# cmaestre/pcl_tracking

Hardware: NVIDIA B200
Metric: likelihood evals/s (particle x model-point), 217k-pt scene tracker frame (higher is better)
Workload: dtype f32

## Files before the change

include/pft/pft.h:

```cpp
#ifndef PFT_PFT_H_
#define PFT_PFT_H_

#include <stddef.h>
#include <stdint.h>

#ifdef __cplusplus
extern "C" {
#endif

#define PFT_API __attribute__((visibility("default")))

typedef enum {
  PFT_OK = 0,
  PFT_ERR_INVALID = -1,
  PFT_ERR_CUDA = -2,
  PFT_ERR_STATE = -3,
  PFT_ERR_CAPACITY = -4,
  PFT_ERR_COMM = -5
} pft_status;

typedef struct { float x, y, z; uint32_t rgba; } pft_point;
typedef struct { float x, y, z, w; uint32_t rgba; uint32_t pad[3]; } pft_point_pcl32;
typedef struct { float x, y, z, one, roll, pitch, yaw, weight; } pft_particle;

// ... 50 lines not shown
  PFT_SAMPLER = 7,
  PFT_QUAT_SAMPLE = 8,
  PFT_USE_NORMAL = 9,
  PFT_MIN_INDICES = 10,
  PFT_DEBUG_NN = 11,
  PFT_CANDIDATE_LISTS = 12,
  PFT_USE_CHANGE_DETECTOR = 13,
  PFT_CHANGE_DETECTOR_INTERVAL = 14,
  PFT_CHANGE_DETECTOR_MIN_POINTS = 15,
  PFT_DELTA = 20,
  PFT_EPSILON = 21,
  PFT_ALPHA = 22,
  PFT_MOTION_RATIO = 23,
  PFT_MAX_DIST = 24,
  PFT_DIST_WEIGHT = 25,
  PFT_HSV_WEIGHT = 26,
  PFT_H_WEIGHT = 27, PFT_S_WEIGHT = 28, PFT_V_WEIGHT = 29,
  PFT_SEARCH_RESOLUTION = 30,
  PFT_RESAMPLE_LIKELIHOOD_THR = 31,
  PFT_CHANGE_DETECTOR_RESOLUTION = 32,
  PFT_STEP_NOISE_COV = 40,
  PFT_INIT_NOISE_COV = 41,
  PFT_INIT_NOISE_MEAN = 42,
  PFT_BIN_SIZE = 43
} pft_key;

typedef enum {
  PFT_NN_EXACT = 0,
  PFT_NN_PCL_APPROX = 1
} pft_nn_mode;
typedef enum { PFT_SAMPLER_ALIAS_PCL = 0, PFT_SAMPLER_CDF = 1, PFT_SAMPLER_CDF_VDC = 2 } pft_sampler;

PFT_API int pft_tracker_create(pft_context* ctx, int kld, pft_tracker** out);
PFT_API void pft_tracker_destroy(pft_tracker* t);
PFT_API int pft_tracker_set_i(pft_tracker* t, int key, int value);
PFT_API int pft_tracker_set_d(pft_tracker* t, int key, double value);
PFT_API int pft_tracker_set_vec6(pft_tracker* t, int key, const double* v6);
PFT_API int pft_tracker_set_trans(pft_tracker* t, const float* m12);
PFT_API int pft_tracker_set_reference_cloud(pft_tracker* t, const pft_cloud* cloud);
PFT_API int pft_tracker_set_reference_points(pft_tracker* t, const void* host_points, size_t n, int layout);
PFT_API int pft_tracker_set_input_cloud(pft_tracker* t, const pft_cloud* cloud);

PFT_API int pft_tracker_compute(pft_tracker* t);
PFT_API int pft_compute_batch(pft_tracker** trackers, int n);
PFT_API int pft_tracker_get_result(pft_tracker* t, pft_particle* out);
PFT_API int pft_tracker_get_particles(pft_tracker* t, pft_particle* out, size_t capacity, size_t* n);
PFT_API int pft_particle_to_matrix(pft_context* ctx, const pft_particle* p, float* m12);
typedef struct {
  float centroid[3];
  float axes[9];
  float extent[3];
  float center[3];
  float quat[4];
  float eigenvalues[3];
  int32_t n;
} pft_result_box;
PFT_API int pft_tracker_get_result_box(pft_tracker* t, float z_offset, pft_result_box* out);
PFT_API int pft_tracker_reset(pft_tracker* t);
PFT_API int pft_tracker_get_eval_count(pft_tracker* t, uint64_t* out);
PFT_API int pft_tracker_get_fit_ratio(pft_tracker* t, double* out);

PFT_API int pft_tracker_set_particles(pft_tracker* t, const pft_particle* p, size_t n);
PFT_API int pft_tracker_set_result(pft_tracker* t, const pft_particle* representative, const pft_particle* motion);
PFT_API int pft_tracker_get_motion(pft_tracker* t, pft_particle* out);
PFT_API int pft_tracker_inject_draws(pft_tracker* t, const float* u_select, const float* normals6,
                                     const float* u_motion, int slots, int stride);
PFT_API int pft_tracker_seed(pft_tracker* t, uint64_t seed);
PFT_API int pft_tracker_init_particles(pft_tracker* t);
PFT_API int pft_tracker_resample(pft_tracker* t, int slot);
PFT_API int pft_tracker_weight(pft_tracker* t);
PFT_API int pft_tracker_update(pft_tracker* t);
PFT_API int pft_tracker_set_changed(pft_tracker* t, int changed);
PFT_API int pft_tracker_get_change_detector_info(pft_tracker* t, int32_t* out4);
PFT_API int pft_tracker_get_aabb(pft_tracker* t, float* aabb6);
PFT_API int pft_tracker_get_cropped_count(pft_tracker* t, size_t* n);
PFT_API int pft_tracker_get_raw_weights(pft_tracker* t, float* out, size_t capacity, size_t* n);
PFT_API int pft_tracker_get_ancestors(pft_tracker* t, int32_t* out, size_t capacity, size_t* n);
PFT_API int pft_tracker_get_nn(pft_tracker* t, int particle, int32_t* idx, float* d2, size_t capacity);
PFT_API int pft_tracker_get_timing(pft_tracker* t, float* weight_kernel_ms, float* compute_ms);
PFT_API int pft_tracker_enable_timing(pft_tracker* t, int on);
PFT_API int pft_tracker_get_kernel_times(pft_tracker* t, const char** names, float* ms, int capacity, int* n);

PFT_API int pft_tracker_get_index_info(pft_tracker* t, int* info8);
PFT_API int pft_tracker_graph_replays(pft_tracker* t, uint64_t* n);

PFT_API int pft_tracker_weight_phase(pft_tracker* t, int phase);
PFT_API int pft_tracker_get_crop_box(pft_tracker* t, float* aabb6);
PFT_API int pft_tracker_set_crop_box(pft_tracker* t, const float* aabb6);
PFT_API int pft_tracker_get_raw_slice(pft_tracker* t, int rank, float* out, size_t capacity, size_t* n);
PFT_API int pft_tracker_set_raw_slice(pft_tracker* t, int rank, const float* in, size_t n);
PFT_API int pft_tracker_set_shard(pft_tracker* t, int nranks, int rank);

PFT_API int pft_comm_get_unique_id(void* id128);
PFT_API int pft_context_comm_init(pft_context* ctx, int nranks, int rank, const void* id128);
PFT_API int pft_context_comm_destroy(pft_context* ctx);
PFT_API int pft_cloud_broadcast(pft_cloud* cloud, size_t capacity, int root);
PFT_API int pft_tracker_comm_init(pft_tracker* t, int nranks, int rank, const void* id128);
PFT_API int pft_tracker_comm_destroy(pft_tracker* t);


#define PFT_PEER_HANDLE_BYTES 64
PFT_API int pft_tracker_peer_export(pft_tracker* t, void* handle64);
PFT_API int pft_tracker_peer_attach(pft_tracker* t, const void* handles );
PFT_API int pft_tracker_peer_detach(pft_tracker* t);

#define PFT_CLOUD_PEER_HANDLE_BYTES 192
PFT_API int pft_cloud_peer_export(pft_cloud* cloud, size_t capacity, void* handles192);
PFT_API int pft_cloud_peer_attach(pft_cloud* cloud, const void* handles , int nranks, int rank);
PFT_API int pft_cloud_peer_broadcast(pft_cloud* cloud, int root);
PFT_API int pft_cloud_peer_detach(pft_cloud* cloud);

PFT_API int pft_tracker_set_devices(pft_tracker* t, int n, const int* devices);
PFT_API int pft_tracker_get_follower(pft_tracker* t, int rank, pft_tracker** out);

#ifdef __cplusplus
}
#endif
#endif
```

pcl_tracking_b200/_capi.py:

```python
import ctypes as C
import os

import numpy as np

_HERE = os.path.dirname(os.path.abspath(__file__))
LIB_PATH = os.environ.get("PFT_LIB") or os.path.join(_HERE, "lib", "libpft.so")
HEADER_PATH = os.path.join(os.path.dirname(_HERE), "include", "pft", "pft.h")

POINT = np.dtype([("x", "<f4"), ("y", "<f4"), ("z", "<f4"), ("rgba", "<u4")])
POINT_PCL32 = np.dtype([("x", "<f4"), ("y", "<f4"), ("z", "<f4"), ("w", "<f4"), ("rgba", "<u4"), ("pad", "<u4", (3,))])
PARTICLE = np.dtype([("x", "<f4"), ("y", "<f4"), ("z", "<f4"), ("one", "<f4"),
                     ("roll", "<f4"), ("pitch", "<f4"), ("yaw", "<f4"), ("weight", "<f4")])

RESULT_BOX = np.dtype([("centroid", "<f4", (3,)), ("axes", "<f4", (3, 3)), ("extent", "<f4", (3,)), ("center", "<f4", (3,)),
                       ("quat", "<f4", (4,)), ("eigenvalues", "<f4", (3,)), ("n", "<i4")])

LAYOUT_PACKED16, LAYOUT_PCL32 = 0, 1
OK, ERR_INVALID, ERR_CUDA, ERR_STATE, ERR_CAPACITY, ERR_COMM = 0, -1, -2, -3, -4, -5

THREADS, PARTICLE_NUM, MAX_PARTICLE_NUM, ITERATION_NUM, NN_MODE, USE_HSV, USE_DISTANCE, SAMPLER, QUAT_SAMPLE, USE_NORMAL, MIN_INDICES, DEBUG_NN, CANDIDATE_LISTS = range(13)
(DELTA, EPSILON, ALPHA, MOTION_RATIO, MAX_DIST, DIST_WEIGHT, HSV_WEIGHT, H_WEIGHT, S_WEIGHT, V_WEIGHT, SEARCH_RESOLUTION,
 RESAMPLE_LIKELIHOOD_THR) = range(20, 32)
STEP_NOISE_COV, INIT_NOISE_COV, INIT_NOISE_MEAN, BIN_SIZE = range(40, 44)
USE_CHANGE_DETECTOR, CHANGE_DETECTOR_INTERVAL, CHANGE_DETECTOR_MIN_POINTS = 13, 14, 15
CHANGE_DETECTOR_RESOLUTION = 32
NN_EXACT, NN_PCL_APPROX = 0, 1
PEER_HANDLE_BYTES = 64
CLOUD_PEER_HANDLE_BYTES = 192
SAMPLER_ALIAS_PCL, SAMPLER_CDF, SAMPLER_CDF_VDC = 0, 1, 2


class PftError(RuntimeError):
    def __init__(self, code, msg):
        super().__init__("pft error %d: %s" % (code, msg))
        self.code = code


_vp, _i, _f, _d, _sz, _u64 = C.c_void_p, C.c_int, C.c_float, C.c_double, C.c_size_t, C.c_uint64
_pp = C.POINTER(C.c_void_p)
_psz = C.POINTER(C.c_size_t)

SIGNATURES = {
    "pft_last_error": (C.c_char_p, []),
    "pft_version": (C.c_char_p, []),
    "pft_device_count": (_i, []),
    "pft_context_create": (_i, [_i, _pp]),
    "pft_context_destroy": (None, [_vp]),
    "pft_context_synchronize": (_i, [_vp]),
    "pft_context_stream": (_vp, [_vp]),
    "pft_host_alloc": (_i, [_pp, _sz]),
    "pft_host_free": (_i, [_vp]),
    "pft_kernel_launch_count": (_u64, []),
    "pft_cloud_create": (_i, [_vp, _pp]),
    "pft_cloud_destroy": (None, [_vp]),
    "pft_cloud_upload": (_i, [_vp, _vp, _sz, _i]),
    "pft_cloud_upload_pointcloud2": (_i, [_vp, _vp, C.c_uint32, C.c_uint32, C.c_uint32, C.c_uint32, C.c_int32, C.c_int32, C.c_int32, C.c_int32, _i]),
    "pft_cloud_upload_async": (_i, [_vp, _vp, _sz, _i]),
    "pft_cloud_upload_pointcloud2_async": (_i, [_vp, _vp, C.c_uint32, C.c_uint32, C.c_uint32, C.c_uint32, C.c_int32, C.c_int32, C.c_int32, C.c_int32, _i]),
    "pft_cloud_wait_upload": (_i, [_vp]),
    "pft_cloud_size": (_i, [_vp, _psz]),
    "pft_cloud_download": (_i, [_vp, _vp, _sz, _i, _psz]),
    "pft_passthrough": (_i, [_vp, _vp, _vp, _i, _f, _f]),
    "pft_passthrough_voxel_grid": (_i, [_vp, _vp, _vp, _f, _i, _f, _f]),
    "pft_approx_voxel_grid_pcl": (_i, [_vp, _vp, _vp, _f, _i, _f, _f]),
    "pft_prepare_model": (_i, [_vp, _vp, _vp, _f, _vp]),
    "pft_euclidean_clusters": (_i, [_vp, _vp, _d, _i, _i, _vp, _sz, _vp, _sz, _psz]),
    "pft_cloud_select_cluster": (_i, [_vp, _vp, _i, _vp]),
    "pft_segment_plane": (_i, [_vp, _vp, _d, _i, _d, _vp, _i, _u64, _i, _vp, C.POINTER(C.c_int32), _vp, _vp, _psz]),
    "pft_tracker_create": (_i, [_vp, _i, _pp]),
    "pft_tracker_destroy": (None, [_vp]),
    "pft_tracker_set_i": (_i, [_vp, _i, _i]),
    "pft_tracker_set_d": (_i, [_vp, _i, _d]),
    "pft_tracker_set_vec6": (_i, [_vp, _i, _vp]),
    "pft_tracker_set_trans": (_i, [_vp, _vp]),
    "pft_tracker_set_reference_cloud": (_i, [_vp, _vp]),
    "pft_tracker_set_reference_points": (_i, [_vp, _vp, _sz, _i]),
    "pft_tracker_set_input_cloud": (_i, [_vp, _vp]),
    "pft_tracker_compute": (_i, [_vp]),
    "pft_compute_batch": (_i, [_pp, _i]),
    "pft_tracker_get_result": (_i, [_vp, _vp]),
    "pft_tracker_get_particles": (_i, [_vp, _vp, _sz, _psz]),
    "pft_particle_to_matrix": (_i, [_vp, _vp, _vp]),
    "pft_tracker_get_result_box": (_i, [_vp, _f, _vp]),
    "pft_tracker_reset": (_i, [_vp]),
    "pft_tracker_get_eval_count": (_i, [_vp, C.POINTER(C.c_uint64)]),
    "pft_tracker_get_fit_ratio": (_i, [_vp, C.POINTER(C.c_double)]),
    "pft_tracker_set_particles": (_i, [_vp, _vp, _sz]),
    "pft_tracker_set_result": (_i, [_vp, _vp, _vp]),
    "pft_tracker_get_motion": (_i, [_vp, _vp]),
    "pft_tracker_inject_draws": (_i, [_vp, _vp, _vp, _vp, _i, _i]),
    "pft_tracker_seed": (_i, [_vp, _u64]),
    "pft_tracker_init_particles": (_i, [_vp]),
    "pft_tracker_resample": (_i, [_vp, _i]),
    "pft_tracker_weight": (_i, [_vp]),
    "pft_tracker_update": (_i, [_vp]),
    "pft_tracker_set_changed": (_i, [_vp, _i]),
    "pft_tracker_get_change_detector_info": (_i, [_vp, _vp]),
    "pft_tracker_get_aabb": (_i, [_vp, _vp]),
    "pft_tracker_get_cropped_count": (_i, [_vp, _psz]),
    "pft_tracker_get_raw_weights": (_i, [_vp, _vp, _sz, _psz]),
    "pft_tracker_get_ancestors": (_i, [_vp, _vp, _sz, _psz]),
    "pft_tracker_get_nn": (_i, [_vp, _i, _vp, _vp, _sz]),
    "pft_tracker_get_timing": (_i, [_vp, C.POINTER(C.c_float), C.POINTER(C.c_float)]),
    "pft_tracker_enable_timing": (_i, [_vp, _i]),
    "pft_tracker_get_kernel_times": (_i, [_vp, _vp, _vp, _i, C.POINTER(C.c_int)]),
    "pft_tracker_get_index_info": (_i, [_vp, _vp]),
    "pft_tracker_graph_replays": (_i, [_vp, C.POINTER(C.c_uint64)]),
    "pft_tracker_weight_phase": (_i, [_vp, _i]),
    "pft_tracker_get_crop_box": (_i, [_vp, _vp]),
    "pft_tracker_set_crop_box": (_i, [_vp, _vp]),
    "pft_tracker_get_raw_slice": (_i, [_vp, _i, _vp, _sz, _psz]),
    "pft_tracker_set_raw_slice": (_i, [_vp, _i, _vp, _sz]),
    "pft_tracker_set_shard": (_i, [_vp, _i, _i]),
    "pft_comm_get_unique_id": (_i, [_vp]),
    "pft_context_comm_init": (_i, [_vp, _i, _i, _vp]),
    "pft_context_comm_destroy": (_i, [_vp]),
    "pft_cloud_broadcast": (_i, [_vp, _sz, _i]),
    "pft_tracker_comm_init": (_i, [_vp, _i, _i, _vp]),
    "pft_tracker_comm_destroy": (_i, [_vp]),
    "pft_cloud_peer_export": (_i, [_vp, _sz, _vp]),
    "pft_cloud_peer_attach": (_i, [_vp, _vp, _i, _i]),
    "pft_cloud_peer_broadcast": (_i, [_vp, _i]),
    "pft_cloud_peer_detach": (_i, [_vp]),
    "pft_tracker_set_devices": (_i, [_vp, _i, _vp]),
    "pft_tracker_get_follower": (_i, [_vp, _i, _vp]),
    "pft_tracker_peer_export": (_i, [_vp, _vp]),
    "pft_tracker_peer_attach": (_i, [_vp, _vp]),
    "pft_tracker_peer_detach": (_i, [_vp]),
}

_lib = None


def load():
    global _lib
    if _lib is None:
        if not os.path.exists(LIB_PATH):
            raise ImportError(
                "%s is missing: build it with `python -m pcl_tracking_b200.build` (nvcc, sm_100a). "
                "There is no CPU fallback." % LIB_PATH)
        L = C.CDLL(LIB_PATH)
        for name, (res, args) in SIGNATURES.items():
            fn = getattr(L, name)
            fn.restype = res
            fn.argtypes = args
        _lib = L
    return _lib


def check(rc):
    if rc != 0:
        raise PftError(rc, load().pft_last_error().decode("utf-8", "replace"))


def ptr(a):
    return a.ctypes.data_as(C.c_void_p)
```

pcl_tracking_b200/csrc/pft_filters.cu:

```cuda
#include <stdlib.h>
#include <string.h>

#include "pft_internal.h"

namespace pft {

namespace {

constexpr unsigned long long kEmptyKey = ~0ull;
constexpr int kFirstInit = 0x7f7f7f7f;

__device__ __forceinline__ bool finite3(const float4& p) { return isfinite(p.x) && isfinite(p.y) && isfinite(p.z); }

__device__ __forceinline__ bool passes(const float4& p, int field, float lo, float hi) {
  if (!finite3(p)) return false;
  if (field < 0) return true;
  const float v = field == 0 ? p.x : (field == 1 ? p.y : p.z);
  return !(v < lo || v > hi);
}

__device__ __forceinline__ unsigned long long voxel_key(const float4& p, float inv) {
  const int ix = (int)floorf(p.x * inv), iy = (int)floorf(p.y * inv), iz = (int)floorf(p.z * inv);
  const unsigned long long bx = (unsigned long long)((ix + (1 << 20)) & 0x1fffff);
  const unsigned long long by = (unsigned long long)((iy + (1 << 20)) & 0x1fffff);
  const unsigned long long bz = (unsigned long long)((iz + (1 << 20)) & 0x1fffff);
  return (bx << 42) | (by << 21) | bz;
}
__device__ __forceinline__ unsigned int hash_key(unsigned long long k) {
  k ^= k >> 33; k *= 0xff51afd7ed558ccdull; k ^= k >> 33; k *= 0xc4ceb9fe1a85ec53ull; k ^= k >> 33;
  return (unsigned int)k;
}

__global__ void unpack_pcl32_kernel(const uint4* __restrict__ src, float4* __restrict__ dst, size_t n) {
  for (size_t i = blockIdx.x * (size_t)blockDim.x + threadIdx.x; i < n; i += (size_t)gridDim.x * blockDim.x) {
    const uint4 a = src[2 * i];
    const uint4 b = src[2 * i + 1];
    dst[i] = make_float4(__uint_as_float(a.x), __uint_as_float(a.y), __uint_as_float(a.z), __uint_as_float(b.x));
  }
}
__global__ void pack_pcl32_kernel(const float4* __restrict__ src, uint4* __restrict__ dst, size_t n) {
  for (size_t i = blockIdx.x * (size_t)blockDim.x + threadIdx.x; i < n; i += (size_t)gridDim.x * blockDim.x) {
    const float4 p = src[i];
    dst[2 * i] = make_uint4(__float_as_uint(p.x), __float_as_uint(p.y), __float_as_uint(p.z), __float_as_uint(1.0f));
    dst[2 * i + 1] = make_uint4(__float_as_uint(p.w), 0u, 0u, 0u);
  }
}
__global__ void unpack_pointcloud2_kernel(const unsigned int* __restrict__ src, float4* __restrict__ dst, unsigned int width, unsigned int height,
                                          unsigned int point_words, unsigned int row_words, int wx, int wy, int wz, int wrgb) {
  const size_t n = (size_t)width * height;
  for (size_t i = blockIdx.x * (size_t)blockDim.x + threadIdx.x; i < n; i += (size_t)gridDim.x * blockDim.x) {
    const size_t row = i / width, col = i - row * width;
    const unsigned int* rec = src + row * row_words + col * point_words;
    const unsigned int rgba = wrgb >= 0 ? rec[wrgb] : 0u;
    dst[i] = make_float4(__uint_as_float(rec[wx]), __uint_as_float(rec[wy]), __uint_as_float(rec[wz]), __uint_as_float(rgba));
  }
}
__global__ void set_header_kernel(CloudHeader* h, int n) { h->n = n; }

__global__ void __launch_bounds__(1024) passthrough_kernel(const float4* __restrict__ in, const CloudHeader* __restrict__ in_hdr,
                                                           float4* __restrict__ out, CloudHeader* out_hdr, int field, float lo,
                                                           float hi, int drop_zero) {
  __shared__ int smem[34];
  const int n = in_hdr->n;
  auto keep = [&](int i) -> int {
    const float4 p = in[i];
    if (!passes(p, field, lo, hi)) return 0;
    if (drop_zero && fabs((double)p.x) < 0.01 && fabs((double)p.y) < 0.01 && fabs((double)p.z) < 0.01) return 0;
    return 1;
  };
  const int total = block_exclusive_scan<int>(
      n, keep, [&](int i, int ex) { const float4 p = in[i]; if (keep(i)) out[ex] = p; }, smem);
  if (threadIdx.x == 0) out_hdr->n = total;
}

__global__ void k1_insert_kernel(const float4* __restrict__ in, const CloudHeader* __restrict__ in_hdr, unsigned long long* keys,
                                 int* first, int* __restrict__ slot_of, unsigned int mask, float inv, int field, float lo, float hi) {
  const int n = in_hdr->n;
  for (int i = blockIdx.x * blockDim.x + threadIdx.x; i < n; i += gridDim.x * blockDim.x) {
    const float4 p = in[i];
    int slot = -1;
    if (passes(p, field, lo, hi)) {
      const unsigned long long key = voxel_key(p, inv);
      unsigned int s = hash_key(key) & mask;
      while (true) {
        const unsigned long long prev = atomicCAS(&keys[s], kEmptyKey, key);
        if (prev == kEmptyKey || prev == key) break;
        s = (s + 1) & mask;
      }
      slot = (int)s;
      atomicMin(&first[s], i);
    }
    slot_of[i] = slot;
  }
}
constexpr int kTile = 4096;

__device__ __forceinline__ int k1_is_first(int i, int n, const int* __restrict__ slot_of, const int* __restrict__ first) {
  if (i >= n) return 0;
  const int s = slot_of[i];
  return (s >= 0 && first[s] == i) ? 1 : 0;
}
__global__ void __launch_bounds__(1024) k1_tile_count_kernel(const CloudHeader* __restrict__ in_hdr, const int* __restrict__ slot_of,
                                                             const int* __restrict__ first, int* __restrict__ tile_count) {
  __shared__ int red[32];
  const int n = in_hdr->n;
  const int base = blockIdx.x * kTile + threadIdx.x * 4;
  int c = 0;
#pragma unroll
  for (int k = 0; k < 4; ++k) c += k1_is_first(base + k, n, slot_of, first);
  c = warp_sum(c);
  if ((threadIdx.x & 31) == 0) red[threadIdx.x >> 5] = c;
  __syncthreads();
  if (threadIdx.x < 32) {
    int v = red[threadIdx.x];
    v = warp_sum(v);
    if (threadIdx.x == 0) tile_count[blockIdx.x] = v;
  }
}
__global__ void __launch_bounds__(1024) k1_tile_scan_kernel(int n_tiles, int* tile_count, CloudHeader* out_hdr) {
  __shared__ int smem[34];
  const int total = block_exclusive_scan<int>(
      n_tiles, [&](int i) { return tile_count[i]; }, [&](int i, int ex) { tile_count[i] = ex; }, smem);
  if (threadIdx.x == 0) out_hdr->n = total;
}
__global__ void __launch_bounds__(1024) k1_tile_assign_kernel(const CloudHeader* __restrict__ in_hdr, const int* __restrict__ slot_of,
                                                              const int* __restrict__ first, const int* __restrict__ tile_offset,
                                                              int* __restrict__ vid, double* acc_xyz, unsigned int* acc_rgbc) {
  __shared__ int wsum[32];
  const int n = in_hdr->n;
  const int lane = threadIdx.x & 31, wid = threadIdx.x >> 5;
  const int base = blockIdx.x * kTile + threadIdx.x * 4;
  int f[4], sum = 0;
#pragma unroll
  for (int k = 0; k < 4; ++k) { f[k] = k1_is_first(base + k, n, slot_of, first); sum += f[k]; }
  int inc = sum;
#pragma unroll
  for (int o = 1; o < 32; o <<= 1) { const int t = __shfl_up_sync(kFull, inc, o); if (lane >= o) inc += t; }
  if (lane == 31) wsum[wid] = inc;
  __syncthreads();
  if (wid == 0) {
    const int w = wsum[lane];
    int winc = w;
#pragma unroll
    for (int o = 1; o < 32; o <<= 1) { const int t = __shfl_up_sync(kFull, winc, o); if (lane >= o) winc += t; }
    wsum[lane] = winc - w;
  }
  __syncthreads();
  int ex = tile_offset[blockIdx.x] + wsum[wid] + (inc - sum);
#pragma unroll
  for (int k = 0; k < 4; ++k) {
    if (f[k]) {
      vid[slot_of[base + k]] = ex;
      ++ex;
    }
  }
}
__global__ void k1_accum_kernel(const float4* __restrict__ in, const CloudHeader* __restrict__ in_hdr, const int* __restrict__ slot_of,
                                const int* __restrict__ vid, double* acc_xyz, unsigned int* acc_rgbc) {
  const int n = in_hdr->n;
  for (int i = blockIdx.x * blockDim.x + threadIdx.x; i < n; i += gridDim.x * blockDim.x) {
    const int s = slot_of[i];
    if (s < 0) continue;
    const int v = vid[s];
    const float4 p = in[i];
    const unsigned int rgba = __float_as_uint(p.w);
    atomicAdd(&acc_xyz[3 * v], (double)p.x);
    atomicAdd(&acc_xyz[3 * v + 1], (double)p.y);
    atomicAdd(&acc_xyz[3 * v + 2], (double)p.z);
    atomicAdd(&acc_rgbc[4 * v], (rgba >> 16) & 0xffu);
    atomicAdd(&acc_rgbc[4 * v + 1], (rgba >> 8) & 0xffu);
    atomicAdd(&acc_rgbc[4 * v + 2], rgba & 0xffu);
    atomicAdd(&acc_rgbc[4 * v + 3], 1u);
  }
}
__global__ void k1_final_kernel(const CloudHeader* __restrict__ out_hdr, const double* __restrict__ acc_xyz,
                                const unsigned int* __restrict__ acc_rgbc, float4* __restrict__ out) {
  const int n = out_hdr->n;
  for (int v = blockIdx.x * blockDim.x + threadIdx.x; v < n; v += gridDim.x * blockDim.x) {
    const uint4 c = reinterpret_cast<const uint4*>(acc_rgbc)[v];
    const double cnt = (double)c.w;
    const float fc = (float)c.w;
    const unsigned int r = (unsigned int)(int)((float)c.x / fc), g = (unsigned int)(int)((float)c.y / fc), b = (unsigned int)(int)((float)c.z / fc);
    out[v] = make_float4((float)(acc_xyz[3 * v] / cnt), (float)(acc_xyz[3 * v + 1] / cnt), (float)(acc_xyz[3 * v + 2] / cnt),
                         __uint_as_float((r << 16) | (g << 8) | b));
  }
}

__global__ void approx_voxel_grid_pcl_kernel(const float4* __restrict__ in, const CloudHeader* __restrict__ in_hdr, float inv, int field, float lo,
                                             float hi, float4* __restrict__ out, CloudHeader* out_hdr) {
  if (threadIdx.x != 0 || blockIdx.x != 0) return;
  constexpr int kHist = 512;
  __shared__ int s_key[kHist][4];
  __shared__ float s_acc[kHist][6];
  for (int k = 0; k < kHist; ++k) { s_key[k][3] = 0; for (int q = 0; q < 6; ++q) s_acc[k][q] = 0.f; }
  const int n = in_hdr->n;
  int op = 0;
  auto flush = [&](int k) {
    const float cnt = (float)s_key[k][3];
    const unsigned int r = (unsigned int)(int)(s_acc[k][3] / cnt), g = (unsigned int)(int)(s_acc[k][4] / cnt), b = (unsigned int)(int)(s_acc[k][5] / cnt);
    out[op++] = make_float4(s_acc[k][0] / cnt, s_acc[k][1] / cnt, s_acc[k][2] / cnt, __uint_as_float((r << 16) | (g << 8) | b));
  };
  for (int i = 0; i < n; ++i) {
    const float4 p = in[i];
    if (!passes(p, field, lo, hi)) continue;
    const int ix = (int)floorf(p.x * inv), iy = (int)floorf(p.y * inv), iz = (int)floorf(p.z * inv);
    const int k = (int)((unsigned int)(ix * 7171 + iy * 3079 + iz * 4231) & (unsigned int)(kHist - 1));
    if (s_key[k][3] && (ix != s_key[k][0] || iy != s_key[k][1] || iz != s_key[k][2])) {
      flush(k);
      s_key[k][3] = 0;
      for (int q = 0; q < 6; ++q) s_acc[k][q] = 0.f;
    }
    s_key[k][0] = ix; s_key[k][1] = iy; s_key[k][2] = iz; s_key[k][3]++;
    const unsigned int rgba = __float_as_uint(p.w);
    s_acc[k][0] += p.x; s_acc[k][1] += p.y; s_acc[k][2] += p.z;
    s_acc[k][3] += (float)((rgba >> 16) & 0xffu); s_acc[k][4] += (float)((rgba >> 8) & 0xffu); s_acc[k][5] += (float)(rgba & 0xffu);
  }
  for (int k = 0; k < kHist; ++k) if (s_key[k][3]) flush(k);
  out_hdr->n = op;
}

__global__ void __launch_bounds__(1024) centre_kernel(float4* pts, const CloudHeader* __restrict__ hdr, float* centroid3) {
  __shared__ double red[32];
  __shared__ float c[3];
  const int n = hdr->n;
  double sx = 0, sy = 0, sz = 0;
  for (int i = threadIdx.x; i < n; i += blockDim.x) { const float4 p = pts[i]; sx += (double)p.x; sy += (double)p.y; sz += (double)p.z; }
  sx = block_sum(sx, red); sy = block_sum(sy, red); sz = block_sum(sz, red);
  if (threadIdx.x == 0) {
    const double dn = n > 0 ? (double)n : 1.0;
    c[0] = (float)(sx / dn); c[1] = (float)(sy / dn); c[2] = (float)(sz / dn);
    centroid3[0] = c[0]; centroid3[1] = c[1]; centroid3[2] = c[2];
  }
  __syncthreads();
  for (int i = threadIdx.x; i < n; i += blockDim.x) { float4 p = pts[i]; p.x = p.x - c[0]; p.y = p.y - c[1]; p.z = p.z - c[2]; pts[i] = p; }
}

inline int grid_for(size_t n, int block, int sm_count) {
  size_t g = (n + block - 1) / block;
  size_t cap = (size_t)sm_count * 8;
  if (g > cap) g = cap;
  if (g < 1) g = 1;
  return (int)g;
}

}

int launch_unpack_pcl32(cudaStream_t s, const void* src32, float4* dst, size_t n) {
  if (n == 0) return PFT_OK;
  unpack_pcl32_kernel<<<grid_for(n, 256, 148), 256, 0, s>>>(reinterpret_cast<const uint4*>(src32), dst, n);
  PFT_LAUNCH_CHECK();
  return PFT_OK;
}
int launch_unpack_pointcloud2(cudaStream_t s, const void* src, float4* dst, unsigned int width, unsigned int height, unsigned int point_step,
                              unsigned int row_step, int off_x, int off_y, int off_z, int off_rgb) {
  const size_t n = (size_t)width * height;
  if (n == 0) return PFT_OK;
  unpack_pointcloud2_kernel<<<grid_for(n, 256, 148), 256, 0, s>>>(reinterpret_cast<const unsigned int*>(src), dst, width, height, point_step / 4, row_step / 4,
                                                                 off_x / 4, off_y / 4, off_z / 4, off_rgb >= 0 ? off_rgb / 4 : -1);
  PFT_LAUNCH_CHECK();
  return PFT_OK;
}
int launch_pack_pcl32(cudaStream_t s, const float4* src, void* dst32, size_t n) {
  if (n == 0) return PFT_OK;
  pack_pcl32_kernel<<<grid_for(n, 256, 148), 256, 0, s>>>(src, reinterpret_cast<uint4*>(dst32), n);
  PFT_LAUNCH_CHECK();
  return PFT_OK;
}
int launch_set_header(cudaStream_t s, CloudHeader* hdr, int n) {
  set_header_kernel<<<1, 1, 0, s>>>(hdr, n);
  PFT_LAUNCH_CHECK();
  return PFT_OK;
}

int run_passthrough(pft_context* ctx, const pft_cloud* in, pft_cloud* out, int field, float lo, float hi, int drop_zero) {
  int rc = out->ensure(in->capacity);
  if (rc) return rc;
  passthrough_kernel<<<1, 1024, 0, ctx->stream>>>(in->d_pts(), in->d_hdr(), out->d_pts(), out->d_hdr(), field, lo, hi, drop_zero);
  PFT_LAUNCH_CHECK();
  out->host_n = -1;
  return PFT_OK;
}

static int enqueue_voxel_grid(pft_context* ctx, const pft_cloud* in, pft_cloud* out, float leaf, int field, float lo, float hi, size_t cap, size_t H,
                              int n_tiles) {
  cudaStream_t s = ctx->stream;
  PFT_CUDA_TRY(cudaMemsetAsync(ctx->k1_keys.p, 0xff, H * sizeof(unsigned long long), s));
  PFT_CUDA_TRY(cudaMemsetAsync(ctx->k1_first.p, 0x7f, H * sizeof(int), s));
  PFT_CUDA_TRY(cudaMemsetAsync(ctx->k1_acc_xyz.p, 0, cap * 3 * sizeof(double), s));
  PFT_CUDA_TRY(cudaMemsetAsync(ctx->k1_acc_rgbc.p, 0, cap * 4 * sizeof(unsigned int), s));
  const float inv = 1.0f / leaf;
  const int grid = grid_for(cap, 256, ctx->sm_count);
  k1_insert_kernel<<<grid, 256, 0, s>>>(in->d_pts(), in->d_hdr(), ctx->k1_keys.as<unsigned long long>(), ctx->k1_first.as<int>(),
                                        ctx->k1_slot_of.as<int>(), (unsigned int)(H - 1), inv, field, lo, hi);
  PFT_LAUNCH_CHECK();
  k1_tile_count_kernel<<<n_tiles, 1024, 0, s>>>(in->d_hdr(), ctx->k1_slot_of.as<int>(), ctx->k1_first.as<int>(), ctx->k1_blk.as<int>());
  PFT_LAUNCH_CHECK();
  k1_tile_scan_kernel<<<1, 1024, 0, s>>>(n_tiles, ctx->k1_blk.as<int>(), out->d_hdr());
  PFT_LAUNCH_CHECK();
  k1_tile_assign_kernel<<<n_tiles, 1024, 0, s>>>(in->d_hdr(), ctx->k1_slot_of.as<int>(), ctx->k1_first.as<int>(), ctx->k1_blk.as<int>(),
                                                 ctx->k1_vid.as<int>(), ctx->k1_acc_xyz.as<double>(), ctx->k1_acc_rgbc.as<unsigned int>());
  PFT_LAUNCH_CHECK();
  k1_accum_kernel<<<grid, 256, 0, s>>>(in->d_pts(), in->d_hdr(), ctx->k1_slot_of.as<int>(), ctx->k1_vid.as<int>(),
                                       ctx->k1_acc_xyz.as<double>(), ctx->k1_acc_rgbc.as<unsigned int>());
  PFT_LAUNCH_CHECK();
  k1_final_kernel<<<grid, 256, 0, s>>>(out->d_hdr(), ctx->k1_acc_xyz.as<double>(), ctx->k1_acc_rgbc.as<unsigned int>(), out->d_pts());
  PFT_LAUNCH_CHECK();
  return PFT_OK;
}

int run_voxel_grid(pft_context* ctx, const pft_cloud* in, pft_cloud* out, float leaf, int field, float lo, float hi) {
  if (!(leaf > 0.f)) { set_last_error("leaf size must be positive"); return PFT_ERR_INVALID; }
  const size_t cap = in->capacity;
  int rc = out->ensure(cap);
  if (rc) return rc;
  if (cap == 0) return launch_set_header(ctx->stream, out->d_hdr(), 0);
  size_t H = 1024;
  while (H < 2 * cap) H <<= 1;
  if ((rc = ctx->k1_keys.reserve(H * sizeof(unsigned long long)))) return rc;
  if ((rc = ctx->k1_first.reserve(H * sizeof(int)))) return rc;
  if ((rc = ctx->k1_vid.reserve(H * sizeof(int)))) return rc;
  if ((rc = ctx->k1_slot_of.reserve(cap * sizeof(int)))) return rc;
  if ((rc = ctx->k1_acc_xyz.reserve(cap * 3 * sizeof(double)))) return rc;
  if ((rc = ctx->k1_acc_rgbc.reserve(cap * 4 * sizeof(unsigned int)))) return rc;
  const int n_tiles = (int)((cap + kTile - 1) / kTile);
  if ((rc = ctx->k1_blk.reserve((size_t)n_tiles * sizeof(int)))) return rc;
  out->host_n = -1;
  (void)kFirstInit;
  static const bool use_graph = [] { const char* e = getenv("PFT_NO_GRAPH"); return !(e && e[0] == '1'); }();
  if (!use_graph) return enqueue_voxel_grid(ctx, in, out, leaf, field, lo, hi, cap, H, n_tiles);
  pft_context::K1Key key;
  memset(&key, 0, sizeof(key));
  key.p[0] = in->d_pts(); key.p[1] = in->d_hdr(); key.p[2] = out->d_pts(); key.p[3] = out->d_hdr();
  key.p[4] = ctx->k1_keys.p; key.p[5] = ctx->k1_first.p; key.p[6] = ctx->k1_vid.p; key.p[7] = ctx->k1_slot_of.p;
  key.p[8] = ctx->k1_acc_xyz.p; key.p[9] = ctx->k1_acc_rgbc.p; key.p[10] = ctx->k1_blk.p;
  key.cap = cap; key.H = H; key.leaf = leaf; key.lo = lo; key.hi = hi; key.field = field;
  int slot = -1;
  for (int k = 0; k < pft_context::kK1Graphs; ++k)
    if (ctx->k1_exec[k] && memcmp(&ctx->k1_key[k], &key, sizeof(key)) == 0) { slot = k; break; }
  if (slot < 0) {
    slot = ctx->k1_next;
    ctx->k1_next = (ctx->k1_next + 1) % pft_context::kK1Graphs;
    if (ctx->k1_exec[slot]) { cudaGraphExecDestroy(ctx->k1_exec[slot]); ctx->k1_exec[slot] = nullptr; }
    cudaGraph_t graph = nullptr;
    const unsigned long long before = g_launch_count.load();
    PFT_CUDA_TRY(cudaStreamBeginCapture(ctx->stream, cudaStreamCaptureModeThreadLocal));
    rc = enqueue_voxel_grid(ctx, in, out, leaf, field, lo, hi, cap, H, n_tiles);
    cudaError_t ce = cudaStreamEndCapture(ctx->stream, &graph);
    g_launch_count -= g_launch_count.load() - before;
    if (rc) { if (graph) cudaGraphDestroy(graph); return rc; }
    if (ce != cudaSuccess) { set_last_error("downsample graph capture failed: %s", cudaGetErrorString(ce)); cudaGetLastError(); return PFT_ERR_CUDA; }
    cudaError_t ie = cudaGraphInstantiate(&ctx->k1_exec[slot], graph, 0);
    cudaGraphDestroy(graph);
    if (ie != cudaSuccess) { set_last_error("downsample graph instantiate failed: %s", cudaGetErrorString(ie)); cudaGetLastError(); ctx->k1_exec[slot] = nullptr; return PFT_ERR_CUDA; }
    ctx->k1_key[slot] = key;
  }
  PFT_CUDA_TRY(cudaGraphLaunch(ctx->k1_exec[slot], ctx->stream));
  g_launch_count += 6;
  return PFT_OK;
}

int run_approx_voxel_grid_pcl(pft_context* ctx, const pft_cloud* in, pft_cloud* out, float leaf, int field, float lo, float hi) {
  if (!(leaf > 0.f)) { set_last_error("leaf size must be positive"); return PFT_ERR_INVALID; }
  int rc = out->ensure(in->capacity);
  if (rc) return rc;
  approx_voxel_grid_pcl_kernel<<<1, 32, 0, ctx->stream>>>(in->d_pts(), in->d_hdr(), 1.0f / leaf, field, lo, hi, out->d_pts(), out->d_hdr());
  PFT_LAUNCH_CHECK();
  out->host_n = -1;
  return PFT_OK;
}

int run_centre_on_centroid(pft_context* ctx, pft_cloud* cloud, float* d_centroid3) {
  centre_kernel<<<1, 1024, 0, ctx->stream>>>(cloud->d_pts(), cloud->d_hdr(), d_centroid3);
  PFT_LAUNCH_CHECK();
  return PFT_OK;
}

}
```

pcl_tracking_b200/csrc/pft_tracker.cu:

```cuda
#include <dlfcn.h>
#include <math.h>
#include <stdio.h>
#include <stdlib.h>
#include <string.h>

#include <algorithm>
#include <vector>

#include "pft_internal.h"
#include "pft_tracker_kernels.cuh"

using namespace pft;

namespace {

struct UidByValue { char internal[128]; };
struct NcclApi {
  void* lib = nullptr;
  bool tried = false;
  int (*GetUniqueId)(void*) = nullptr;
  int (*CommInitRank)(void**, int, UidByValue, int) = nullptr;
  int (*CommDestroy)(void*) = nullptr;
  int (*AllGather)(const void*, void*, size_t, int, void*, cudaStream_t) = nullptr;
  int (*Broadcast)(const void*, void*, size_t, int, int, void*, cudaStream_t) = nullptr;
// ... 23 lines not shown
  g_nccl.GetUniqueId = (decltype(g_nccl.GetUniqueId))sym("ncclGetUniqueId");
  g_nccl.CommInitRank = (decltype(g_nccl.CommInitRank))sym("ncclCommInitRank");
  g_nccl.CommDestroy = (decltype(g_nccl.CommDestroy))sym("ncclCommDestroy");
  g_nccl.AllGather = (decltype(g_nccl.AllGather))sym("ncclAllGather");
  g_nccl.AllReduce = (decltype(g_nccl.AllReduce))sym("ncclAllReduce");
  g_nccl.Broadcast = (decltype(g_nccl.Broadcast))sym("ncclBroadcast");
  g_nccl.GroupStart = (decltype(g_nccl.GroupStart))sym("ncclGroupStart");
  g_nccl.GroupEnd = (decltype(g_nccl.GroupEnd))sym("ncclGroupEnd");
  g_nccl.GetErrorString = (decltype(g_nccl.GetErrorString))sym("ncclGetErrorString");
  if (!g_nccl.GetUniqueId || !g_nccl.CommInitRank || !g_nccl.CommDestroy || !g_nccl.AllGather || !g_nccl.AllReduce || !g_nccl.Broadcast || !g_nccl.GroupStart ||
      !g_nccl.GroupEnd) {
    set_last_error("NCCL library lacks a required symbol");
    return PFT_ERR_COMM;
  }
  g_nccl.lib = h;
  return PFT_OK;
}
#define PFT_NCCL_TRY(expr)                                                                                       \
  do {                                                                                                           \
    int _r = (expr);                                                                                             \
    if (_r != 0) {                                                                                               \
      set_last_error("%s:%d: %s -> %s", __FILE__, __LINE__, #expr, g_nccl.GetErrorString ? g_nccl.GetErrorString(_r) : "nccl error"); \
      return PFT_ERR_COMM;                                                                                       \
    }                                                                                                            \
  } while (0)

inline int blocks_for(long long n, int block, int cap) {
  long long g = (n + block - 1) / block;
  if (g > cap) g = cap;
  if (g < 1) g = 1;
  return (int)g;
}

}

struct pft_tracker {
  pft_context* ctx = nullptr;
  bool kld = true;
  int threads = 0, particle_num = 0, max_particle_num = 0, iteration_num = 1, min_indices = 1;
  int nn_mode = PFT_NN_EXACT, use_hsv = 0, use_dist = 1, sampler = PFT_SAMPLER_CDF, quat_sample = 1, debug_nn = 0;
  double delta = 0.99, epsilon = 0.0, alpha = 15.0, motion_ratio = 0.25, max_dist = 1.79769313486231570815e+308;
  double dist_w = 1.0, hsv_w = 1.0, h_w = 1.0, s_w = 1.0, v_w = 0.0, search_res = 0.01, resample_thr = 0.0;
  double step_cov[6] = {0, 0, 0, 0, 0, 0}, init_cov[6] = {0, 0, 0, 0, 0, 0}, init_mean[6] = {0, 0, 0, 0, 0, 0};
  float bin_size[6] = {0, 0, 0, 0, 0, 0};
  float trans[12] = {1, 0, 0, 0, 0, 1, 0, 0, 0, 0, 1, 0};
  unsigned long long seed = 0x5eedull;
  bool changed = false, has_particles = false;
  int n_cap = 0;
  int M = 0;
  const pft_cloud* input = nullptr;
  size_t scene_cap = 0;
  int max_cells = 1 << 20;
  int list_mode = 1;
  int list_max_cells = 1 << 19;
  int cur = 0;
  int inj_slots = 0, inj_stride = 0;
  int draw_cap = 0;
  bool timing = false;
  float t_weight_ms = 0.f, t_compute_ms = 0.f;
  std::vector<cudaEvent_t> ev_w;
  cudaEvent_t ev_c0 = nullptr, ev_c1 = nullptr;
  int n_ev_used = 0;
  std::vector<cudaEvent_t> ev_k;
  std::vector<const char*> ev_k_name;
  int n_ev_k = 0;
  void* comm = nullptr;
  int nranks = 1, rank = 0;
  bool peer_mode = false;
  bool peer_ipc = true;
  struct Follower { pft_context* ctx = nullptr; pft_tracker* t = nullptr; pft_cloud* scene = nullptr; pft_cloud* model = nullptr; cudaEvent_t scene_ready = nullptr, scene_free = nullptr; bool free_recorded = false; };
  std::vector<Follower> followers;
  bool md_attached = false, md_prepared = false;
  void* peer_local = nullptr;
  size_t peer_bytes = 0;
  PeerSet peers{};
  bool graph_enabled = true;
  cudaGraphExec_t graph_exec[2] = {nullptr, nullptr};
  const void* graph_scene_pts[2] = {nullptr, nullptr};
  const void* graph_scene_hdr[2] = {nullptr, nullptr};
  unsigned long long config_version = 1, graph_version[2] = {0, 0};
  unsigned long long graph_replays = 0;
  int graph_nodes[2] = {0, 0};
  DevBuf st, parts[2], mats, slot_aabb, model, model_perm, model_tmp, sort_keys, sort_idx, bbox, raw, partial, cdf, cdf_total, ancestors, bin_keys, tbl_rep,
      tbl_min, slot_of, klb, d_usel, d_normals, d_umot, idx_hdr, idx_hdr_prev, fbuilt_bits, cell_start, ipts, ipts2, ihsv, icount, dbg_idx, dbg_d2, d_trans, row_table, flists, fpool, fcell_items, fl1_slots, fneeded, fneeded_list, ffar_list, xlists, xcount, result_box, alias_a, alias_q, alias_hl, oct_hdr, oct_nodes, oct_next, cd_hdr, cd_nodes, cd_out;
  int oct_node_cap = 0;
  bool use_cd = false;
  int cd_interval = 10, cd_filter = 10, change_counter = 0, cd_tests = 0, cd_last_found = -1, cd_node_cap = 0, cd_resets = 0;
  double cd_res = 0.01;
  int lists_smem = 0;
  int tbl_size = 0;
  int n_slots = 0;
  int chunks = 1, chunk_len = 0;

  cudaStream_t aux_stream = nullptr;
  cudaEvent_t ev_fork = nullptr, ev_join = nullptr;
  cudaStream_t batch_stream = nullptr;
  cudaEvent_t batch_done = nullptr;
  bool batch_active = false;

  int slice_cap() const { return (n_cap + nranks - 1) / nranks; }
  cudaStream_t run_stream() const { return batch_active ? batch_stream : ctx->stream; }
};

namespace {

void invalidate_graph(pft_tracker* t) { t->config_version++; }

void stage_mark(pft_tracker* t, const char* name) {
  if (!t->timing) return;
  if ((int)t->ev_k.size() <= t->n_ev_k) {
    cudaEvent_t e;
    if (cudaEventCreate(&e) != cudaSuccess) return;
    t->ev_k.push_back(e);
    t->ev_k_name.push_back(name);
  }
  t->ev_k_name[t->n_ev_k] = name;
  cudaEventRecord(t->ev_k[t->n_ev_k++], t->run_stream());
}

void release_all(pft_tracker* t) {
  DevBuf* bufs[] = {&t->st, &t->parts[0], &t->parts[1], &t->mats, &t->slot_aabb, &t->model, &t->model_perm, &t->model_tmp, &t->sort_keys, &t->sort_idx,
                    &t->bbox, &t->raw, &t->partial, &t->cdf, &t->cdf_total, &t->ancestors, &t->bin_keys, &t->tbl_rep, &t->tbl_min, &t->slot_of, &t->klb,
                    &t->d_usel, &t->d_normals, &t->d_umot, &t->idx_hdr, &t->idx_hdr_prev, &t->fbuilt_bits, &t->cell_start, &t->ipts, &t->ipts2, &t->ihsv, &t->icount, &t->dbg_idx,
                    &t->dbg_d2, &t->d_trans, &t->row_table, &t->flists, &t->fpool, &t->fcell_items, &t->fl1_slots, &t->fneeded, &t->fneeded_list, &t->ffar_list, &t->xlists, &t->xcount, &t->result_box, &t->alias_a, &t->alias_q, &t->alias_hl, &t->oct_hdr, &t->oct_nodes, &t->oct_next, &t->cd_hdr, &t->cd_nodes, &t->cd_out};
  for (auto* b : bufs) b->release();
}

NoiseParams make_noise(const pft_tracker* t, const double* mean, const double* cov) {
  NoiseParams np;
  for (int d = 0; d < 6; ++d) { np.mean[d] = mean[d]; np.sigma[d] = sqrt(cov[d]); }
  const float scale_factor = 0.2862f;
  for (int d = 0; d < 3; ++d) np.sigma_q[d] = sqrt((double)scale_factor * cov[3 + d]);
  np.quat_mode = t->quat_sample;
  return np;
}

double normal_quantile(double u) {
  static const double a[9] = {1.24818987e-4, -1.075204047e-3, 5.198775019e-3, -0.019198292004, 0.059054035642,
                              -0.151968751364, 0.319152932694, -0.5319230073, 0.797884560593};
  static const double b[15] = {-4.5255659e-5, 1.5252929e-4, -1.9538132e-5, -6.76904986e-4, 1.390604284e-3,
                               -7.9462082e-4, -2.034254874e-3, 6.549791214e-3, -0.010557625006, 0.011630447319,
                               -9.279453341e-3, 5.353579108e-3, -2.141268741e-3, 5.35310549e-4, 0.999936657524};
  if (u == 0.) return 0.5;
  double y = u / 2.0, z;
  if (y < -3.) return 0.0;
  if (y > 3.) return 1.0;
  if (y < 0.0) y = -y;
  if (y < 1.0) {
    const double w = y * y;
    z = a[0];
    for (int i = 1; i < 9; i++) z = z * w + a[i];
    z *= (y * 2.0);
  } else {
    y -= 2.0;
    z = b[0];
    for (int i = 1; i < 15; i++) z = z * y + b[i];
  }
  return u < 0.0 ? (1.0 - z) / 2.0 : (1.0 + z) / 2.0;
}
double kl_bound(int k, double delta, double eps) {
  const double z = normal_quantile(delta);
  const double chi = 1.0 - 2.0 / (9.0 * (k - 1)) + sqrt(2.0 / (9.0 * (k - 1))) * z;
  return ((k - 1.0) / (2.0 * eps)) * chi * chi * chi;
}

constexpr long long kMarkCountMaxQueries = 16ll << 20;
constexpr int kClusterMinParticles = 4096;
constexpr int kListThreads = 640;
constexpr int kListThreadsBig = 896;
constexpr long long kListBigQueries = 48ll << 20;
constexpr long long kDynItemsPerWarp = 5;
constexpr int kItemsPerWarp = 6;
constexpr int kChunkWarpsPerSm = 24;
constexpr float kIndexDilate = 0.03f;
constexpr int kListRatio = 2;

template <typename... P, typename... A>
void launch_replicated(const pft_tracker* t, void (*one)(P...), void (*cluster)(P...), A... args) {
  if (t->n_cap > kClusterMinParticles) cluster<<<kClusterCtas, 1024, 0, t->run_stream()>>>(args...);
  else one<<<1, 1024, 0, t->run_stream()>>>(args...);
}

int upload_row_table(pft_tracker* t) {
  std::vector<RowEntry> tab;
  tab.reserve(kRows);
  for (int dz = -kRT; dz <= kRT; ++dz)
    for (int dy = -kRT; dy <= kRT; ++dy) {
      const int gy = std::max(std::abs(dy) - 1, 0), gz = std::max(std::abs(dz) - 1, 0);
      tab.push_back(RowEntry{(signed char)dy, (signed char)dz, (unsigned short)(gy * gy + gz * gz)});
    }
  std::stable_sort(tab.begin(), tab.end(), [](const RowEntry& a, const RowEntry& b) {
    if (a.lb2 != b.lb2) return a.lb2 < b.lb2;
    return (a.dy * a.dy + a.dz * a.dz) < (b.dy * b.dy + b.dz * b.dz);
  });
  int rc = t->row_table.reserve(tab.size() * sizeof(RowEntry));
  if (rc) return rc;
  PFT_CUDA_TRY(cudaMemcpyAsync(t->row_table.p, tab.data(), tab.size() * sizeof(RowEntry), cudaMemcpyHostToDevice, t->run_stream()));
  PFT_CUDA_TRY(cudaStreamSynchronize(t->run_stream()));
  int dev = t->ctx->device, max_optin = 0;
  PFT_CUDA_TRY(cudaDeviceGetAttribute(&max_optin, cudaDevAttrMaxSharedMemoryPerBlockOptin, dev));
  cudaFuncAttributes fa;
  PFT_CUDA_TRY(cudaFuncGetAttributes(&fa, weight_lists_kernel<true, kListThreads, true>));
  int dyn_l = (max_optin - (int)fa.sharedSizeBytes - 1024) & ~15;
  if (dyn_l < 0) dyn_l = 0;
  PFT_CUDA_TRY(cudaFuncSetAttribute(weight_lists_kernel<true, kListThreads, true>, cudaFuncAttributeMaxDynamicSharedMemorySize, dyn_l));
  PFT_CUDA_TRY(cudaFuncSetAttribute(weight_lists_kernel<true, kListThreads, false>, cudaFuncAttributeMaxDynamicSharedMemorySize, dyn_l));
  PFT_CUDA_TRY(cudaFuncSetAttribute(weight_lists_kernel<false, kListThreads, true>, cudaFuncAttributeMaxDynamicSharedMemorySize, dyn_l));
  PFT_CUDA_TRY(cudaFuncSetAttribute(weight_lists_kernel<false, kListThreads, false>, cudaFuncAttributeMaxDynamicSharedMemorySize, dyn_l));
  PFT_CUDA_TRY(cudaFuncSetAttribute(weight_lists_kernel<true, kListThreadsBig, true>, cudaFuncAttributeMaxDynamicSharedMemorySize, dyn_l));
  PFT_CUDA_TRY(cudaFuncSetAttribute(weight_lists_kernel<false, kListThreadsBig, true>, cudaFuncAttributeMaxDynamicSharedMemorySize, dyn_l));
  t->lists_smem = dyn_l;
  if (t->list_max_cells / 8 + 64 > max_optin - 2048) t->list_max_cells = (max_optin - 4096) * 8;
  PFT_CUDA_TRY(cudaFuncSetAttribute(cand_mark_kernel<false>, cudaFuncAttributeMaxDynamicSharedMemorySize, t->list_max_cells / 8 + 64));
  PFT_CUDA_TRY(cudaFuncSetAttribute(cand_mark_kernel<true>, cudaFuncAttributeMaxDynamicSharedMemorySize, t->list_max_cells / 8 + 64));
  return PFT_OK;
}

int upload_kl_table(pft_tracker* t);

int wanted_cap(const pft_tracker* t) { return t->kld ? std::max(t->max_particle_num, t->particle_num) : t->particle_num; }

int ensure_particle_buffers(pft_tracker* t) {
  const int cap = std::max(wanted_cap(t), t->n_cap);
  if (cap <= 0) { set_last_error("particle count is zero: call setParticleNum / setMaximumParticleNum first"); return PFT_ERR_STATE; }
  cudaStream_t s = t->run_stream();
  int rc;
  if (!t->st.p) {
    if ((rc = t->st.reserve(sizeof(TrackerState)))) return rc;
    PFT_CUDA_TRY(cudaMemsetAsync(t->st.p, 0, sizeof(TrackerState), s));
    DevParticle one{0.f, 0.f, 0.f, 1.f, 0.f, 0.f, 0.f, 0.f};
    PFT_CUDA_TRY(cudaMemcpyAsync(&t->st.as<TrackerState>()->rep, &one, sizeof(one), cudaMemcpyHostToDevice, s));
    PFT_CUDA_TRY(cudaMemcpyAsync(&t->st.as<TrackerState>()->motion, &one, sizeof(one), cudaMemcpyHostToDevice, s));
    PFT_CUDA_TRY(cudaStreamSynchronize(s));
    if ((rc = t->cdf_total.reserve(sizeof(unsigned long long)))) return rc;
    if ((rc = t->idx_hdr.reserve(sizeof(IndexHeader)))) return rc;
    if ((rc = t->idx_hdr_prev.reserve(sizeof(IndexHeader)))) return rc;
    PFT_CUDA_TRY(cudaMemsetAsync(t->idx_hdr.p, 0, sizeof(IndexHeader), s));
    PFT_CUDA_TRY(cudaMemsetAsync(t->idx_hdr_prev.p, 0, sizeof(IndexHeader), s));
    PFT_CUDA_TRY(cudaStreamSynchronize(s));
    if ((rc = t->d_trans.reserve(12 * sizeof(float)))) return rc;
    if ((rc = t->cell_start.reserve(((size_t)t->max_cells + 16) * sizeof(int)))) return rc;
    if ((rc = t->icount.reserve(((size_t)t->max_cells + 16) * sizeof(int)))) return rc;
    if ((rc = upload_row_table(t))) return rc;
    if (t->list_max_cells > 0) {
      if ((rc = t->flists.reserve(((size_t)t->list_max_cells + 1) * 8 * 8 * sizeof(unsigned int)))) return rc;
      if ((rc = t->fpool.reserve((size_t)kPoolGroups * 8 * sizeof(unsigned int)))) return rc;
      if ((rc = t->fcell_items.reserve(((size_t)t->list_max_cells + 16) * sizeof(int2)))) return rc;
      if ((rc = t->fl1_slots.reserve(((size_t)t->list_max_cells + 1) * kL1Cap * sizeof(unsigned short)))) return rc;
      if ((rc = t->fneeded.reserve(((size_t)t->list_max_cells + 16) * sizeof(unsigned int)))) return rc;
      if ((rc = t->fbuilt_bits.reserve(((size_t)t->list_max_cells / 32 + 16) * sizeof(unsigned int)))) return rc;
      if ((rc = t->fneeded_list.reserve(((size_t)t->list_max_cells / 2 + 4096) * sizeof(int)))) return rc;
      if ((rc = t->ffar_list.reserve(((size_t)t->list_max_cells + 16) * sizeof(int)))) return rc;
      if ((rc = t->xlists.reserve((size_t)kListXCells * kListKX * sizeof(unsigned int)))) return rc;
      if ((rc = t->xcount.reserve(64))) return rc;
    }
  }
  if (cap == t->n_cap) return PFT_OK;
  if (t->peer_local) {
    set_last_error("the particle capacity (%d -> %d) cannot change once the peer window is exported", t->n_cap, cap);
    return PFT_ERR_STATE;
  }
  invalidate_graph(t);
  PFT_CUDA_TRY(cudaStreamSynchronize(s));
  const int old_cap = t->n_cap;
  DevBuf np0, np1;
  if ((rc = np0.reserve((size_t)cap * sizeof(DevParticle)))) return rc;
  if ((rc = np1.reserve((size_t)cap * sizeof(DevParticle)))) return rc;
  if (old_cap > 0 && t->has_particles) {
    PFT_CUDA_TRY(cudaMemcpyAsync(np0.p, t->parts[t->cur].p, (size_t)std::min(cap, old_cap) * sizeof(DevParticle), cudaMemcpyDeviceToDevice, s));
    PFT_CUDA_TRY(cudaStreamSynchronize(s));
  }
  t->parts[0].release(); t->parts[1].release();
  t->parts[0] = np0; t->parts[1] = np1; t->cur = 0;
  t->n_cap = cap;
  t->n_slots = cap;
  const int slice = t->slice_cap();
  if ((rc = t->mats.reserve((size_t)cap * 12 * sizeof(float)))) return rc;
  t->slot_aabb.release();
  if ((rc = t->slot_aabb.reserve((size_t)cap * 6 * sizeof(float)))) return rc;
  {
    std::vector<float> init((size_t)cap * 6);
    for (int i = 0; i < cap; ++i) { for (int d = 0; d < 3; ++d) { init[6 * i + d] = FLT_MAX; init[6 * i + 3 + d] = -FLT_MAX; } }
    PFT_CUDA_TRY(cudaMemcpyAsync(t->slot_aabb.p, init.data(), init.size() * sizeof(float), cudaMemcpyHostToDevice, s));
    PFT_CUDA_TRY(cudaStreamSynchronize(s));
  }
  if ((rc = t->raw.reserve((size_t)slice * t->nranks * sizeof(float)))) return rc;
  PFT_CUDA_TRY(cudaMemsetAsync(t->raw.p, 0, (size_t)slice * t->nranks * sizeof(float), s));
  if ((rc = t->cdf.reserve((size_t)cap * sizeof(unsigned long long)))) return rc;
  if ((rc = t->ancestors.reserve((size_t)cap * sizeof(int)))) return rc;
  PFT_CUDA_TRY(cudaMemsetAsync(t->ancestors.p, 0xff, (size_t)cap * sizeof(int), s));
  PFT_CUDA_TRY(cudaStreamSynchronize(s));
  if (t->kld) {
    if ((rc = t->bin_keys.reserve((size_t)cap * 6 * sizeof(int)))) return rc;
    int ts = 1024;
    while (ts < 2 * cap) ts <<= 1;
    t->tbl_size = ts;
    if ((rc = t->tbl_rep.reserve((size_t)ts * sizeof(int)))) return rc;
    if ((rc = t->tbl_min.reserve((size_t)ts * sizeof(int)))) return rc;
    if ((rc = t->slot_of.reserve((size_t)cap * sizeof(int)))) return rc;
    if ((rc = t->klb.reserve((size_t)(cap + 2) * sizeof(double)))) return rc;
    if ((rc = upload_kl_table(t))) return rc;
  }
  return PFT_OK;
}

int upload_kl_table(pft_tracker* t) {
  if (!t->kld) return PFT_OK;
  const int n = t->n_cap + 2;
  std::vector<double> tab(n, 0.0);
  for (int k = 2; k < n; ++k) tab[k] = kl_bound(k, t->delta, t->epsilon);
  PFT_CUDA_TRY(cudaMemcpyAsync(t->klb.p, tab.data(), tab.size() * sizeof(double), cudaMemcpyHostToDevice, t->run_stream()));
  PFT_CUDA_TRY(cudaStreamSynchronize(t->run_stream()));
  return PFT_OK;
}

int ensure_draw_buffers(pft_tracker* t, int slots, int stride) {
  const size_t n = (size_t)slots * stride;
  int rc;
  if ((rc = t->d_usel.reserve(n * sizeof(float)))) return rc;
  if ((rc = t->d_normals.reserve(n * 6 * sizeof(float)))) return rc;
  if ((rc = t->d_umot.reserve(n * sizeof(float)))) return rc;
  return PFT_OK;
}

int reserve_generated_draws(pft_tracker* t, int count) {
  if (t->draw_cap >= count) return PFT_OK;
  int rc = ensure_draw_buffers(t, 1, count);
  if (rc) return rc;
  t->draw_cap = count;
  invalidate_graph(t);
  return PFT_OK;
}

int prepare_draws(pft_tracker* t, int slot, int count, const float** usel, const float** normals, const float** umot) {
  cudaStream_t s = t->run_stream();
  if (t->inj_stride > 0) {
    if (slot >= t->inj_slots || count > t->inj_stride) {
      set_last_error("injected draws cover %d slots x %d, need slot %d x %d", t->inj_slots, t->inj_stride, slot, count);
      return PFT_ERR_STATE;
    }
    *usel = t->d_usel.as<float>() + (size_t)slot * t->inj_stride;
    *normals = t->d_normals.as<float>() + (size_t)slot * t->inj_stride * 6;
    *umot = t->d_umot.as<float>() + (size_t)slot * t->inj_stride;
    return PFT_OK;
  }
  int rc = reserve_generated_draws(t, count);
  if (rc) return rc;
  draws_kernel<<<blocks_for(count, 256, t->ctx->sm_count * 4), 256, 0, s>>>(t->st.as<TrackerState>(), t->d_usel.as<float>(), t->d_normals.as<float>(),
                                                                        t->d_umot.as<float>(), count, t->seed);
  PFT_LAUNCH_CHECK();
  stage_mark(t, "draws_kernel");
  *usel = t->d_usel.as<float>(); *normals = t->d_normals.as<float>(); *umot = t->d_umot.as<float>();
  return PFT_OK;
}

int ensure_index_buffers(pft_tracker* t) {
  const size_t cap = std::max<size_t>(t->input ? t->input->capacity : 0, 1);
  if (cap <= t->scene_cap) return PFT_OK;
  invalidate_graph(t);
  PFT_CUDA_TRY(cudaStreamSynchronize(t->run_stream()));
  int rc;
  if ((rc = t->ipts.reserve((cap + 4) * sizeof(float4)))) return rc;
  if ((rc = t->ipts2.reserve((cap + 4) * sizeof(float4)))) return rc;
  if ((rc = t->ihsv.reserve((cap + 4) * sizeof(unsigned int)))) return rc;
  t->scene_cap = cap;
  return PFT_OK;
}

void choose_chunks(pft_tracker* t) {
  const int n_expected = std::max(1, (t->particle_num > 0 ? t->particle_num : t->n_cap) / t->nranks);
  const int total_warps = t->ctx->sm_count * kChunkWarpsPerSm;
  const int target_items = total_warps * kItemsPerWarp;
  const int max_chunks = std::max(1, (t->M + 63) / 64);
  int chunks = (target_items + n_expected - 1) / n_expected;
  chunks = std::min(std::max(chunks, 1), std::min(max_chunks, 256));
  int len = (t->M + chunks - 1) / chunks;
  len = ((len + 31) / 32) * 32;
  if (len < 32) len = 32;
  chunks = std::max(1, (t->M + len - 1) / len);
  if (chunks != t->chunks || len != t->chunk_len) invalidate_graph(t);
  t->chunks = chunks;
  t->chunk_len = len;
}

CoherenceParams make_coherence(const pft_tracker* t) {
  CoherenceParams c;
  c.max_d2 = t->max_dist * t->max_dist;
  c.dist_w = t->dist_w; c.hsv_w = t->hsv_w;
  c.h_w = (float)t->h_w; c.s_w = (float)t->s_w; c.v_w = (float)t->v_w;
  c.r_max = (float)std::min(t->max_dist, 1.0e18);
  c.use_dist = t->use_dist; c.use_hsv = t->use_hsv;
  return c;
}

int stage_init_particles(pft_tracker* t) {
  int rc = ensure_particle_buffers(t);
  if (rc) return rc;
  if (t->particle_num <= 0) { set_last_error("setParticleNum was not called"); return PFT_ERR_STATE; }
  if ((rc = upload_kl_table(t))) return rc;
  cudaStream_t s = t->run_stream();
  PFT_CUDA_TRY(cudaMemcpyAsync(t->d_trans.p, t->trans, sizeof(t->trans), cudaMemcpyHostToDevice, s));
  const float *usel, *normals, *umot;
  if ((rc = prepare_draws(t, 0, t->particle_num, &usel, &normals, &umot))) return rc;
  const NoiseParams np = make_noise(t, t->init_mean, t->init_cov);
  init_particles_kernel<<<blocks_for(t->particle_num, 128, 1 << 20), 128, 0, s>>>(t->st.as<TrackerState>(), t->parts[t->cur].as<DevParticle>(),
                                                                                   t->particle_num, t->d_trans.as<float>(), np, normals);
  PFT_LAUNCH_CHECK();
  stage_mark(t, "init_particles_kernel");
  t->has_particles = true;
  return PFT_OK;
}

int stage_resample(pft_tracker* t, int slot) {
  if (!t->has_particles) { set_last_error("resample before particles exist"); return PFT_ERR_STATE; }
  if (!t->input) { set_last_error("resample needs an input cloud (setInputCloud)"); return PFT_ERR_STATE; }
  if (t->kld && t->max_particle_num <= 0) { set_last_error("KLD tracker: setMaximumParticleNum was not called"); return PFT_ERR_STATE; }
  cudaStream_t s = t->run_stream();
  const int count = t->kld ? t->max_particle_num : t->particle_num;
  const float *usel = nullptr, *normals = nullptr, *umot = nullptr;
  int rc = PFT_OK;
  if (t->inj_stride > 0 && (rc = prepare_draws(t, slot, count, &usel, &normals, &umot))) return rc;
  TrackerState* st = t->st.as<TrackerState>();
  const DevParticle* old_parts = t->parts[t->cur].as<DevParticle>();
  DevParticle* new_parts = t->parts[t->cur ^ 1].as<DevParticle>();
  launch_replicated(t, cdf_kernel<1>, cdf_kernel<kClusterCtas>, st, old_parts, t->cdf.as<unsigned long long>(), t->cdf_total.as<unsigned long long>(),
                    t->tbl_rep.as<int>(), t->tbl_min.as<int>(), t->kld ? t->tbl_size : 0, t->kld ? 0 : t->particle_num, t->input->d_hdr());
  PFT_LAUNCH_CHECK();
  stage_mark(t, "cdf_kernel");
  if (t->sampler == PFT_SAMPLER_ALIAS_PCL) {
    alias_table_kernel<<<1, 32, 0, s>>>(st, old_parts, t->alias_a.as<int>(), t->alias_q.as<double>(), t->alias_hl.as<int>());
    PFT_LAUNCH_CHECK();
    stage_mark(t, "alias_table_kernel");
  }
  ResampleArgs a;
  a.alias_a = t->alias_a.as<int>(); a.alias_q = t->alias_q.as<double>();
  a.st = st; a.old_parts = old_parts; a.new_parts = new_parts;
  a.cdf = t->cdf.as<unsigned long long>(); a.cdf_total = t->cdf_total.as<unsigned long long>();
  a.u_select = usel; a.normals = normals; a.u_motion = umot; a.seed = t->seed;
  a.scene_hdr = t->input->d_hdr();
  a.ancestors = t->ancestors.as<int>(); a.bin_keys = t->bin_keys.as<int>();
  const double zero[6] = {0, 0, 0, 0, 0, 0};
  a.np = make_noise(t, zero, t->step_cov);
  a.motion_ratio = t->motion_ratio;
  for (int d = 0; d < 6; ++d) a.bin_size[d] = t->bin_size[d];
  a.kld = t->kld ? 1 : 0; a.n_max = t->max_particle_num; a.sampler = t->sampler; a.n_target = t->particle_num;
  resample_kernel<<<blocks_for(count, 128, t->ctx->sm_count * 16), 128, 0, s>>>(a);
  PFT_LAUNCH_CHECK();
// ... 14 lines not shown
int check_weight_ready(pft_tracker* t) {
  if (!t->has_particles) { set_last_error("weight before particles exist"); return PFT_ERR_STATE; }
  if (!t->input) { set_last_error("weight needs an input cloud (setInputCloud)"); return PFT_ERR_STATE; }
  if (t->M <= 0) { set_last_error("weight needs a reference cloud (setReferenceCloud)"); return PFT_ERR_STATE; }
  return ensure_index_buffers(t);
}

int weight_phase_box(pft_tracker* t) {
  int rc = check_weight_ready(t);
  if (rc) return rc;
  cudaStream_t s = t->run_stream();
  const int sm = t->ctx->sm_count;
  TrackerState* st = t->st.as<TrackerState>();
  DevParticle* parts = t->parts[t->cur].as<DevParticle>();
  matrices_kernel<<<blocks_for(t->n_cap, 128, sm * 8), 128, 0, s>>>(st, parts, t->mats.as<float>());
  PFT_LAUNCH_CHECK();
  stage_mark(t, "matrices_kernel");
  if (t->n_slots <= sm * 32) {
    aabb_kernel<4><<<std::min(t->n_slots, sm * 16), 128, 0, s>>>(st, t->model.as<float4>(), t->M, t->mats.as<float>(), t->slot_aabb.as<float>(), t->n_slots,
                                                                t->nranks, t->rank, t->peers, t->peer_mode ? 1 : 0);
  } else {
    aabb_kernel<1><<<std::min(t->n_slots, sm * 64), 32, 0, s>>>(st, t->model.as<float4>(), t->M, t->mats.as<float>(), t->slot_aabb.as<float>(), t->n_slots,
                                                               t->nranks, t->rank, t->peers, t->peer_mode ? 1 : 0);
  }
  PFT_LAUNCH_CHECK();
  stage_mark(t, "aabb_kernel");
  return PFT_OK;
}

bool nccl_exchange(const pft_tracker* t) { return t->comm && !t->peer_mode; }
bool normalize_sums_partials(const pft_tracker* t) { return t->nranks == 1 || t->peer_mode; }

int weight_comm_box(pft_tracker* t) {
  cudaStream_t s = t->run_stream();
  TrackerState* st = t->st.as<TrackerState>();
  PFT_NCCL_TRY(g_nccl.GroupStart());
  PFT_NCCL_TRY(g_nccl.AllReduce(st->aabb, st->aabb, 3, kNcclFloat, kNcclMin, t->comm, s));
  PFT_NCCL_TRY(g_nccl.AllReduce(st->aabb + 3, st->aabb + 3, 3, kNcclFloat, kNcclMax, t->comm, s));
  PFT_NCCL_TRY(g_nccl.GroupEnd());
  return PFT_OK;
}

template <typename Launch>
int timed_lookup(pft_tracker* t, const char* name, Launch launch) {
  cudaStream_t s = t->run_stream();
  if (t->timing) {
    while ((int)t->ev_w.size() < 2 * (t->n_ev_used + 1)) { cudaEvent_t e; PFT_CUDA_TRY(cudaEventCreate(&e)); t->ev_w.push_back(e); }
    PFT_CUDA_TRY(cudaEventRecord(t->ev_w[2 * t->n_ev_used], s));
  }
  launch();
  PFT_LAUNCH_CHECK();
  stage_mark(t, name);
  if (t->timing) { PFT_CUDA_TRY(cudaEventRecord(t->ev_w[2 * t->n_ev_used + 1], s)); t->n_ev_used++; }
  return PFT_OK;
}

int launch_raw_weights(pft_tracker* t) {
  const int local_cap = t->slice_cap();
  raw_weights_kernel<<<blocks_for(local_cap, 256, t->ctx->sm_count * 4), 256, 0, t->run_stream()>>>(
      t->st.as<TrackerState>(), t->partial.as<double>(), t->chunks, t->n_cap, t->raw.as<float>(), local_cap, t->nranks, t->rank);
  PFT_LAUNCH_CHECK();
  stage_mark(t, "raw_weights_kernel");
  return PFT_OK;
}

int weight_eval_pcl_approx(pft_tracker* t) {
  cudaStream_t s = t->run_stream();
  const int sm = t->ctx->sm_count;
  TrackerState* st = t->st.as<TrackerState>();
  const pft_cloud* in = t->input;
  octree_build_kernel<<<1, 32, 0, s>>>(in->d_pts(), in->d_hdr(), t->idx_hdr.as<IndexHeader>(), t->search_res, t->oct_nodes.as<OctNodeD>(), t->oct_node_cap,
                                       t->oct_next.as<int>(), t->oct_hdr.as<OctHeaderD>());
  PFT_LAUNCH_CHECK();
  stage_mark(t, "octree_build_kernel");
  WeightApproxArgs w;
  w.st = st; w.oct = t->oct_hdr.as<OctHeaderD>(); w.nodes = t->oct_nodes.as<OctNodeD>(); w.next = t->oct_next.as<int>();
  w.scene = in->d_pts(); w.model = t->model.as<float4>(); w.model_perm = t->model_perm.as<int>(); w.M = t->M; w.mats = t->mats.as<float>();
  w.partial = t->partial.as<double>(); w.chunks = t->chunks; w.chunk_len = t->chunk_len; w.n_max = t->n_cap; w.nranks = t->nranks; w.rank_id = t->rank;
  w.co = make_coherence(t);
  w.dbg_k = t->debug_nn; w.dbg_idx = t->dbg_idx.as<int>(); w.dbg_d2 = t->dbg_d2.as<float>();
  return timed_lookup(t, "weight_approx_kernel", [&] { weight_approx_kernel<<<sm * 8, 256, 0, s>>>(w); });
}

int launch_index_begin(pft_tracker* t, bool reuse_allowed = false) {
  const int sm = t->ctx->sm_count;
  const float inv_leaf = 1.0f / (float)t->search_res;
  index_begin_kernel<<<sm, 256, 0, t->run_stream()>>>(t->st.as<TrackerState>(), t->idx_hdr.as<IndexHeader>(), t->icount.as<int>(), inv_leaf, t->max_cells,
                                                      t->list_mode ? t->list_max_cells : 0, t->list_mode == 2 ? 0 : t->M, t->nranks, t->rank,
                                                      t->fneeded.as<unsigned int>(), t->xcount.as<int>(), t->fbuilt_bits.as<unsigned int>(),
                                                      reuse_allowed ? 1 : 0, t->iteration_num > 1 ? kIndexDilate : 0.f, kListRatio, t->idx_hdr_prev.as<IndexHeader>());
  PFT_LAUNCH_CHECK();
  stage_mark(t, "index_begin_kernel");
  return PFT_OK;
}

int weight_phase_eval(pft_tracker* t, bool reuse_allowed = false) {
  int rc = check_weight_ready(t);
  if (rc) return rc;
  cudaStream_t s = t->run_stream();
  const int sm = t->ctx->sm_count;
  TrackerState* st = t->st.as<TrackerState>();
  const pft_cloud* in = t->input;
  const int ncap_scene = (int)std::max<size_t>(in->capacity, 1);
  IndexHeader* hdr = t->idx_hdr.as<IndexHeader>();
  const float inv_leaf = 1.0f / (float)t->search_res;
  const int gscene = blocks_for(ncap_scene, 256, sm * 4);
  const bool lists = t->list_max_cells > 0 && t->list_mode && t->nn_mode == PFT_NN_EXACT;
  if ((rc = launch_index_begin(t, reuse_allowed && lists))) return rc;
  if (lists) {
    cudaStream_t sa = t->aux_stream;
    PFT_CUDA_TRY(cudaEventRecord(t->ev_fork, s));
    PFT_CUDA_TRY(cudaStreamWaitEvent(sa, t->ev_fork, 0));
    const long long n_queries = (long long)std::max(1, (t->particle_num > 0 ? t->particle_num : t->n_cap) / t->nranks) * t->M;
    const size_t mark_smem = (size_t)(t->list_max_cells / 8 + 64);
    if (n_queries <= kMarkCountMaxQueries) cand_mark_kernel<true><<<sm * 3, 256, mark_smem, sa>>>(st, hdr, t->model.as<float4>(), t->M, t->mats.as<float>(), t->fneeded.as<unsigned int>(), t->nranks, t->rank, t->fbuilt_bits.as<unsigned int>());
    else cand_mark_kernel<false><<<sm * 3, 256, mark_smem, sa>>>(st, hdr, t->model.as<float4>(), t->M, t->mats.as<float>(), t->fneeded.as<unsigned int>(), t->nranks, t->rank, t->fbuilt_bits.as<unsigned int>());
    PFT_LAUNCH_CHECK();
    cand_collect_kernel<<<sm * 2, 256, 0, sa>>>(hdr, t->fneeded.as<unsigned int>(), t->fneeded_list.as<int>(), t->xcount.as<int>());
    PFT_LAUNCH_CHECK();
    PFT_CUDA_TRY(cudaEventRecord(t->ev_join, sa));
  }
  index_count_kernel<<<gscene, 256, 0, s>>>(in->d_pts(), in->d_hdr(), hdr, t->icount.as<int>(), t->ipts2.as<float4>());
  PFT_LAUNCH_CHECK();
  stage_mark(t, "index_count_kernel");
  index_scan_kernel<<<1, 1024, 0, s>>>(hdr, t->icount.as<int>(), t->cell_start.as<int>(), st, t->ipts.as<float4>(), t->ipts2.as<float4>(), t->idx_hdr_prev.as<IndexHeader>());
  PFT_LAUNCH_CHECK();
  stage_mark(t, "index_scan_kernel");
  index_scatter_kernel<<<gscene, 256, 0, s>>>(in->d_pts(), in->d_hdr(), hdr, t->cell_start.as<int>(), t->icount.as<int>(), t->ipts.as<float4>(),
                                              t->ihsv.as<unsigned int>(), t->ipts2.as<float4>());
  PFT_LAUNCH_CHECK();
  stage_mark(t, "index_scatter_kernel");
  if (lists) {
    PFT_CUDA_TRY(cudaStreamWaitEvent(s, t->ev_join, 0));
    stage_mark(t, "cand_mark+collect (beside the index)");
    cand_build_kernel<<<sm * 8, 256, 0, s>>>(hdr, t->cell_start.as<int>(), t->ipts.as<float4>(), t->max_dist * t->max_dist, t->flists.as<unsigned int>(),
                                            t->fneeded.as<unsigned int>(), t->fneeded_list.as<int>(), t->xcount.as<int>(), t->ffar_list.as<int>(),
                                            t->fcell_items.as<int2>(), t->fl1_slots.as<unsigned short>(), t->fbuilt_bits.as<unsigned int>());
    PFT_LAUNCH_CHECK();
    stage_mark(t, "cand_build_kernel");
    cand_build_far_kernel<<<sm * 4, 256, 0, s>>>(hdr, t->cell_start.as<int>(), t->ipts.as<float4>(), t->max_dist * t->max_dist,
                                                t->flists.as<unsigned int>(), t->xlists.as<unsigned int>(), t->xcount.as<int>(), t->ffar_list.as<int>(),
                                                t->fneeded.as<unsigned int>(), t->fcell_items.as<int2>(), t->fl1_slots.as<unsigned short>(), t->fbuilt_bits.as<unsigned int>());
    PFT_LAUNCH_CHECK();
    stage_mark(t, "cand_build_far_kernel");
    cand_octant_kernel<<<sm * 8, 256, 0, s>>>(hdr, t->ipts.as<float4>(), t->max_dist * t->max_dist, t->flists.as<unsigned int>(), t->fpool.as<unsigned int>(),
                                             t->xcount.as<int>(), t->fcell_items.as<int2>(), t->fl1_slots.as<unsigned short>());
    PFT_LAUNCH_CHECK();
    stage_mark(t, "cand_octant_kernel");
  }
  if (t->nn_mode == PFT_NN_PCL_APPROX) return weight_eval_pcl_approx(t);
  WeightArgs a;
  a.st = st; a.hdr = hdr; a.pts2 = t->ipts2.as<float4>();
  a.flists = t->flists.as<unsigned int>(); a.pool = t->fpool.as<unsigned int>(); a.xlists = t->xlists.as<unsigned int>();
  a.cell_start = t->cell_start.as<int>(); a.pts = t->ipts.as<float4>();
  a.hsv = t->ihsv.as<unsigned int>(); a.table = t->row_table.as<RowEntry>(); a.smem_bytes = t->lists_smem;
  a.model = t->model.as<float4>(); a.model_perm = t->model_perm.as<int>(); a.M = t->M;
  a.mats = t->mats.as<float>();
  a.partial = t->partial.as<double>(); a.chunks = t->chunks; a.chunk_len = t->chunk_len; a.n_max = t->n_cap;
  a.nranks = t->nranks; a.rank_id = t->rank;
  a.co = make_coherence(t);
  a.dbg_k = t->debug_nn; a.dbg_idx = t->dbg_idx.as<int>(); a.dbg_d2 = t->dbg_d2.as<float>();
  const int wgrid = sm;
  const long long n_local = std::max(1, (t->particle_num > 0 ? t->particle_num : t->n_cap) / t->nranks);
  const bool dyn = n_local * t->chunks >= kDynItemsPerWarp * sm * (kListThreads / 32);
  return timed_lookup(t, "weight_lists_kernel", [&] {
    if (n_local * t->M >= kListBigQueries) {
      if (t->use_hsv) weight_lists_kernel<true, kListThreadsBig, true><<<wgrid, kListThreadsBig, t->lists_smem, s>>>(a);
      else weight_lists_kernel<false, kListThreadsBig, true><<<wgrid, kListThreadsBig, t->lists_smem, s>>>(a);
    } else if (t->use_hsv) {
      if (dyn) weight_lists_kernel<true, kListThreads, true><<<wgrid, kListThreads, t->lists_smem, s>>>(a);
      else weight_lists_kernel<true, kListThreads, false><<<wgrid, kListThreads, t->lists_smem, s>>>(a);
    } else {
      if (dyn) weight_lists_kernel<false, kListThreads, true><<<wgrid, kListThreads, t->lists_smem, s>>>(a);
      else weight_lists_kernel<false, kListThreads, false><<<wgrid, kListThreads, t->lists_smem, s>>>(a);
    }
  });
}

int weight_comm_raw(pft_tracker* t) {
  const int local_cap = t->slice_cap();
  PFT_NCCL_TRY(g_nccl.AllGather(t->raw.as<float>() + (size_t)t->rank * local_cap, t->raw.as<float>(), (size_t)local_cap, kNcclFloat, t->comm,
                                t->run_stream()));
  return PFT_OK;
}

int weight_phase_normalize(pft_tracker* t, bool fuse_update = false) {
  int rc = check_weight_ready(t);
  if (rc) return rc;
  launch_replicated(t, normalize_kernel<1>, normalize_kernel<kClusterCtas>, t->st.as<TrackerState>(), t->parts[t->cur].as<DevParticle>(), t->raw.as<float>(),
                    t->alpha, t->nranks, t->slice_cap(), t->input->d_hdr(), t->M, normalize_sums_partials(t) ? t->partial.as<double>() : nullptr,
                    t->chunks, t->n_cap, fuse_update ? 1 : 0, t->peers);
  PFT_LAUNCH_CHECK();
  stage_mark(t, "normalize_kernel");
  t->changed = true;
  return PFT_OK;
}

int change_detection_test(pft_tracker* t, bool* change) {
  int rc = launch_index_begin(t);
  if (rc) return rc;
  cudaStream_t s = t->run_stream();
  for (int attempt = 0; attempt < 2; ++attempt) {
    change_detect_kernel<<<1, 32, 0, s>>>(t->input->d_pts(), t->input->d_hdr(), t->idx_hdr.as<IndexHeader>(), t->cd_res, t->cd_nodes.as<CdNodeD>(), t->cd_node_cap,
                                          t->cd_hdr.as<CdHeaderD>(), t->cd_filter, t->cd_out.as<int>());
    PFT_LAUNCH_CHECK();
    stage_mark(t, "change_detect_kernel");
    int out[2] = {0, 0};
    PFT_CUDA_TRY(cudaMemcpyAsync(out, t->cd_out.p, sizeof(out), cudaMemcpyDeviceToHost, s));
    PFT_CUDA_TRY(cudaStreamSynchronize(s));
    if (!out[1]) { t->cd_last_found = out[0]; t->cd_tests++; *change = out[0] > 0; return PFT_OK; }
    PFT_CUDA_TRY(cudaMemsetAsync(t->cd_hdr.p, 0, sizeof(CdHeaderD), s));
    t->cd_resets++;
  }
  set_last_error("change detector: the cropped cloud does not fit the node pool");
  return PFT_ERR_CAPACITY;
}

int weight_phase_renormalize(pft_tracker* t) {
  cudaStream_t s = t->run_stream();
  TrackerState* st = t->st.as<TrackerState>();
  DevParticle* parts = t->parts[t->cur].as<DevParticle>();
  weights_to_raw_kernel<<<blocks_for(t->n_cap, 256, t->ctx->sm_count * 4), 256, 0, s>>>(st, parts, t->raw.as<float>(), t->nranks, t->slice_cap());
  PFT_LAUNCH_CHECK();
  stage_mark(t, "weights_to_raw_kernel");
  launch_replicated(t, normalize_kernel<1>, normalize_kernel<kClusterCtas>, st, parts, t->raw.as<float>(), t->alpha, t->nranks, t->slice_cap(),
                    t->input->d_hdr(), 0, nullptr, t->chunks, t->n_cap, 0, t->peers);
  PFT_LAUNCH_CHECK();
  stage_mark(t, "normalize_kernel");
  t->changed = false;
  return PFT_OK;
}

int stage_weight(pft_tracker* t, bool fuse_update = false, bool reuse_allowed = false) {
  int rc;
  if ((rc = weight_phase_box(t))) return rc;
  if (nccl_exchange(t) && (rc = weight_comm_box(t))) return rc;
  if (t->use_cd && t->nranks > 1) { set_last_error("the change detector is not supported on a sharded tracker"); return PFT_ERR_STATE; }
  if (t->use_cd) {
    if (t->change_counter == 0) {
      bool change = true;
      if ((rc = change_detection_test(t, &change))) return rc;
      if (!change) return weight_phase_renormalize(t);
      t->change_counter = t->cd_interval;
    } else {
      --t->change_counter;
    }
  }
  if ((rc = weight_phase_eval(t, reuse_allowed))) return rc;
  if (!normalize_sums_partials(t)) {
    if ((rc = launch_raw_weights(t))) return rc;
    if (nccl_exchange(t) && (rc = weight_comm_raw(t))) return rc;
  }
  return weight_phase_normalize(t, fuse_update);
}

int stage_update(pft_tracker* t) {
  if (!t->has_particles || !t->input) { set_last_error("update before weight"); return PFT_ERR_STATE; }
  launch_replicated(t, update_kernel<1>, update_kernel<kClusterCtas>, t->st.as<TrackerState>(), t->parts[t->cur].as<DevParticle>(), t->input->d_hdr());
  PFT_LAUNCH_CHECK();
  stage_mark(t, "update_kernel");
  return PFT_OK;
}

int enqueue_tracking(pft_tracker* t) {
  int rc;
  for (int it = 0; it < t->iteration_num; ++it) {
    if (t->changed && (rc = stage_resample(t, it))) return rc;
    if ((rc = stage_weight(t, true, it > 0 && !t->use_cd))) return rc;
  }
  return PFT_OK;
}

int prepare_compute(pft_tracker* t) {
  int rc = ensure_particle_buffers(t);
  if (rc) return rc;
  if (t->input && (rc = t->input->join_upload())) return rc;
  if ((rc = ensure_index_buffers(t))) return rc;
  if (t->inj_stride == 0 && (rc = reserve_generated_draws(t, t->n_cap))) return rc;
  if (!t->aux_stream) {
    PFT_CUDA_TRY(cudaStreamCreateWithFlags(&t->aux_stream, cudaStreamNonBlocking));
    PFT_CUDA_TRY(cudaEventCreateWithFlags(&t->ev_fork, cudaEventDisableTiming));
    PFT_CUDA_TRY(cudaEventCreateWithFlags(&t->ev_join, cudaEventDisableTiming));
// ... 284 lines not shown
      const int cur0 = t->cur;
      const bool changed0 = t->changed;
      cudaGraph_t graph = nullptr;
      PFT_CUDA_TRY(cudaStreamBeginCapture(s, cudaStreamCaptureModeThreadLocal));
      const unsigned long long launches_before = g_launch_count.load();
      rc = enqueue_tracking(t);
      cudaError_t ce = cudaStreamEndCapture(s, &graph);
      g_launch_count -= g_launch_count.load() - launches_before;
      if (rc || ce != cudaSuccess) {
        t->cur = cur0; t->changed = changed0;
        if (graph) cudaGraphDestroy(graph);
        if (rc) return rc;
        set_last_error("graph capture failed: %s", cudaGetErrorString(ce)); cudaGetLastError(); return PFT_ERR_CUDA;
      }
      size_t n_nodes = 0;
      cudaGraphGetNodes(graph, nullptr, &n_nodes);
      cudaError_t ie = cudaGraphInstantiate(&t->graph_exec[g], graph, 0);
      cudaGraphDestroy(graph);
      if (ie != cudaSuccess) {
        t->cur = cur0; t->changed = changed0;
        set_last_error("graph instantiate failed: %s", cudaGetErrorString(ie)); cudaGetLastError(); t->graph_exec[g] = nullptr; return PFT_ERR_CUDA;
      }
      t->graph_version[g] = version;
      t->config_version = version;
      t->graph_scene_pts[g] = t->input->d_pts();
      t->graph_scene_hdr[g] = t->input->d_hdr();
      t->graph_nodes[g] = (int)n_nodes;
    } else {
      if (t->iteration_num & 1) t->cur ^= 1;
    }
    PFT_CUDA_TRY(cudaGraphLaunch(t->graph_exec[g], s));
    g_launch_count += (unsigned long long)t->graph_nodes[g];
    t->graph_replays++;
    return PFT_OK;
  }
  rc = enqueue_tracking(t);
  if (rc) return rc;
  if (t->timing) PFT_CUDA_TRY(cudaEventRecord(t->ev_c1, s));
  return PFT_OK;
}

static int copy_cloud_to_device(const pft_cloud* src, pft_cloud* dst, cudaEvent_t ready, cudaEvent_t dst_free) {
  PFT_CUDA_TRY(cudaSetDevice(dst->ctx->device));
  int rc = dst->ensure(std::max<size_t>(src->capacity, 1));
  if (rc) return rc;
  PFT_CUDA_TRY(cudaSetDevice(src->ctx->device));
  if ((rc = src->join_upload())) return rc;
  cudaStream_t ss = src->ctx->stream;
  if (dst_free) PFT_CUDA_TRY(cudaStreamWaitEvent(ss, dst_free, 0));
  PFT_CUDA_TRY(cudaMemcpyPeerAsync(dst->hdr.p, dst->ctx->device, src->hdr.p, src->ctx->device, sizeof(CloudHeader), ss));
  if (src->capacity) PFT_CUDA_TRY(cudaMemcpyPeerAsync(dst->pts.p, dst->ctx->device, src->pts.p, src->ctx->device, src->capacity * sizeof(float4), ss));
  dst->host_n = src->host_n;
  dst->capacity = src->capacity;
  if (ready) {
    PFT_CUDA_TRY(cudaEventRecord(ready, ss));
    PFT_CUDA_TRY(cudaSetDevice(dst->ctx->device));
    PFT_CUDA_TRY(cudaStreamWaitEvent(dst->ctx->stream, ready, 0));
  } else {
    PFT_CUDA_TRY(cudaStreamSynchronize(ss));
  }
  return PFT_OK;
}

static int alloc_peer_window(pft_tracker* t);
static int preload_kernels() {
  static const void* const kernels[] = {
      (const void*)aabb_kernel<1>,
      (const void*)aabb_kernel<4>,
      (const void*)alias_table_kernel,
      (const void*)bitonic_sort_kernel,
      (const void*)cand_build_far_kernel,
      (const void*)cand_build_kernel,
      (const void*)cand_collect_kernel,
      (const void*)cand_mark_kernel<false>,
      (const void*)cand_mark_kernel<true>,
      (const void*)cand_octant_kernel,
      (const void*)cdf_kernel<1>,
      (const void*)cdf_kernel<kClusterCtas>,
      (const void*)change_detect_kernel,
      (const void*)cloud_push_kernel,
      (const void*)cloud_wait_kernel,
      (const void*)draws_kernel,
      (const void*)index_begin_kernel,
      (const void*)index_count_kernel,
      (const void*)index_scan_kernel,
      (const void*)index_scatter_kernel,
      (const void*)init_particles_kernel,
      (const void*)kld_insert_kernel,
      (const void*)kld_stop_kernel,
      (const void*)matrices_kernel,
      (const void*)model_bbox_kernel,
      (const void*)model_gather_kernel,
      (const void*)model_keys_kernel,
      (const void*)normalize_kernel<1>,
      (const void*)normalize_kernel<kClusterCtas>,
      (const void*)octree_build_kernel,
      (const void*)raw_weights_kernel,
      (const void*)resample_kernel,
      (const void*)result_box_kernel,
      (const void*)single_matrix_kernel,
      (const void*)update_kernel<1>,
      (const void*)update_kernel<kClusterCtas>,
      (const void*)weight_approx_kernel,
      (const void*)weight_lists_kernel<false, kListThreads, false>,
      (const void*)weight_lists_kernel<false, kListThreads, true>,
      (const void*)weight_lists_kernel<false, kListThreadsBig, true>,
      (const void*)weight_lists_kernel<true, kListThreads, false>,
      (const void*)weight_lists_kernel<true, kListThreads, true>,
      (const void*)weight_lists_kernel<true, kListThreadsBig, true>,
      (const void*)weights_to_raw_kernel};
  for (const void* k : kernels) {
    cudaFuncAttributes a;
    PFT_CUDA_TRY(cudaFuncGetAttributes(&a, k));
  }
  return PFT_OK;
}

static int compute_multi_device(pft_tracker* t) {
  if (is_noop(t)) return PFT_OK;
  const int n = (int)t->followers.size() + 1;
  int rc;
  if (!t->md_attached) {
    std::vector<pft_tracker*> all{t};
    for (auto& f : t->followers) all.push_back(f.t);
    for (pft_tracker* x : all) {
      PFT_CUDA_TRY(cudaSetDevice(x->ctx->device));
      if ((rc = alloc_peer_window(x))) return rc;
    }
    for (int r = 0; r < n; ++r) {
      PeerSet ps{};
      ps.nranks = n; ps.rank = r;
      for (int q = 0; q < n; ++q) ps.win[q] = reinterpret_cast<PeerWindow*>(all[q]->peer_local);
      all[r]->peers = ps; all[r]->peer_mode = true; all[r]->peer_ipc = false;
      invalidate_graph(all[r]);
    }
    t->md_attached = true;
  }
  for (auto& f : t->followers) {
    if ((rc = copy_cloud_to_device(t->input, f.scene, f.scene_ready, f.free_recorded ? f.scene_free : nullptr))) return rc;
    f.t->input = f.scene;
  }
  {
    std::vector<pft_tracker*> all{t};
    for (auto& f : t->followers) all.push_back(f.t);
    for (pft_tracker* x : all) {
      PFT_CUDA_TRY(cudaSetDevice(x->ctx->device));
      if (!x->md_prepared) { if ((rc = preload_kernels())) return rc; }
      if ((rc = prepare_compute(x))) return rc;
      x->md_prepared = true;
    }
  }
  for (auto& f : t->followers) {
    if ((rc = compute_one(f.t))) return rc;
    PFT_CUDA_TRY(cudaSetDevice(f.ctx->device));
    PFT_CUDA_TRY(cudaEventRecord(f.scene_free, f.ctx->stream));
    f.free_recorded = true;
  }
  return compute_one(t);
}

int pft_tracker_compute(pft_tracker* t) {
  if (!t) { set_last_error("null tracker"); return PFT_ERR_INVALID; }
  if (!t->followers.empty()) return compute_multi_device(t);
  return compute_one(t);
}

int pft_compute_batch(pft_tracker** ts, int n) {
  if (n < 0 || (n && !ts)) { set_last_error("pft_compute_batch: bad arguments"); return PFT_ERR_INVALID; }
  for (int i = 0; i < n; ++i) {
// ... 212 lines not shown
  if (t) for (auto& f_ : t->followers) { int rc_ = pft_tracker_seed(f_.t, seed); if (rc_) return rc_; }
  if (!t) { set_last_error("null tracker"); return PFT_ERR_INVALID; }
  t->seed = seed;
  invalidate_graph(t);
  if (t->st.p) {
    PFT_CUDA_TRY(cudaSetDevice(t->ctx->device));
    PFT_CUDA_TRY(cudaMemsetAsync(&t->st.as<TrackerState>()->draw_call, 0, sizeof(unsigned long long), t->run_stream()));
  }
  return PFT_OK;
}

int pft_tracker_init_particles(pft_tracker* t) {
  if (!t) { set_last_error("null tracker"); return PFT_ERR_INVALID; }
  PFT_CUDA_TRY(cudaSetDevice(t->ctx->device));
  return stage_init_particles(t);
}
int pft_tracker_resample(pft_tracker* t, int slot) {
  if (!t) { set_last_error("null tracker"); return PFT_ERR_INVALID; }
  PFT_CUDA_TRY(cudaSetDevice(t->ctx->device));
  int rc = prepare_compute(t);
  if (rc) return rc;
  return stage_resample(t, slot);
}
int pft_tracker_weight(pft_tracker* t) {
  if (!t) { set_last_error("null tracker"); return PFT_ERR_INVALID; }
  PFT_CUDA_TRY(cudaSetDevice(t->ctx->device));
  int rc = prepare_compute(t);
  if (rc) return rc;
  if (t->timing) t->n_ev_used = 0;
  return stage_weight(t);
}
int pft_tracker_get_change_detector_info(pft_tracker* t, int32_t* out4) {
  if (!t || !out4) { set_last_error("null argument"); return PFT_ERR_INVALID; }
  out4[0] = t->change_counter; out4[1] = t->cd_tests; out4[2] = t->cd_last_found; out4[3] = t->changed ? 1 : 0;
  return PFT_OK;
}
int pft_tracker_update(pft_tracker* t) {
  if (!t) { set_last_error("null tracker"); return PFT_ERR_INVALID; }
  PFT_CUDA_TRY(cudaSetDevice(t->ctx->device));
  return stage_update(t);
}
int pft_tracker_set_changed(pft_tracker* t, int changed) {
  if (t) for (auto& f_ : t->followers) { int rc_ = pft_tracker_set_changed(f_.t, changed); if (rc_) return rc_; }
  if (!t) { set_last_error("null tracker"); return PFT_ERR_INVALID; }
  t->changed = changed != 0;
  return PFT_OK;
}

int pft_tracker_get_aabb(pft_tracker* t, float* aabb6) {
  if (!t || !aabb6) { set_last_error("null argument"); return PFT_ERR_INVALID; }
  if (!t->idx_hdr.p) { set_last_error("no weight() has run"); return PFT_ERR_STATE; }
  PFT_CUDA_TRY(cudaSetDevice(t->ctx->device));
  cudaStream_t s = t->run_stream();
  PFT_CUDA_TRY(cudaMemcpyAsync(t->ctx->pinned, t->idx_hdr.p, sizeof(IndexHeader), cudaMemcpyDeviceToHost, s));
  PFT_CUDA_TRY(cudaStreamSynchronize(s));
  memcpy(aabb6, reinterpret_cast<IndexHeader*>(t->ctx->pinned)->aabb, 6 * sizeof(float));
  return PFT_OK;
}

int pft_tracker_get_cropped_count(pft_tracker* t, size_t* n) {
  if (!t || !n) { set_last_error("null argument"); return PFT_ERR_INVALID; }
  if (!t->idx_hdr.p) { set_last_error("no weight() has run"); return PFT_ERR_STATE; }
  PFT_CUDA_TRY(cudaSetDevice(t->ctx->device));
  cudaStream_t s = t->run_stream();
  PFT_CUDA_TRY(cudaMemcpyAsync(t->ctx->pinned, t->idx_hdr.p, sizeof(IndexHeader), cudaMemcpyDeviceToHost, s));
  PFT_CUDA_TRY(cudaStreamSynchronize(s));
  *n = (size_t)reinterpret_cast<IndexHeader*>(t->ctx->pinned)->n_in_crop;
  return PFT_OK;
}

int pft_tracker_get_index_info(pft_tracker* t, int* info8) {
  if (!t || !info8) { set_last_error("null argument"); return PFT_ERR_INVALID; }
  if (!t->idx_hdr.p) { set_last_error("no weight() has run"); return PFT_ERR_STATE; }
  PFT_CUDA_TRY(cudaSetDevice(t->ctx->device));
  cudaStream_t s = t->run_stream();
  PFT_CUDA_TRY(cudaMemcpyAsync(t->ctx->pinned, t->idx_hdr.p, sizeof(IndexHeader), cudaMemcpyDeviceToHost, s));
  PFT_CUDA_TRY(cudaStreamSynchronize(s));
  const IndexHeader* h = reinterpret_cast<IndexHeader*>(t->ctx->pinned);
  info8[0] = h->dim[0]; info8[1] = h->dim[1]; info8[2] = h->dim[2]; info8[3] = h->level;
  info8[4] = h->n_in_crop; info8[5] = h->n_cells; info8[6] = h->use_lists; info8[7] = h->f_cells;
  return PFT_OK;
}

int pft_tracker_get_raw_weights(pft_tracker* t, float* out, size_t capacity, size_t* n_out) {
  if (!t) { set_last_error("null tracker"); return PFT_ERR_INVALID; }
  TrackerState h;
  int rc = read_state(t, &h);
  if (rc) return rc;
  const size_t n = t->has_particles ? (size_t)h.particle_num : 0;
  if (n_out) *n_out = n;
  if (n > capacity) { set_last_error("capacity %zu < %zu", capacity, n); return PFT_ERR_CAPACITY; }
  if (n == 0) return PFT_OK;
  const int slice = t->slice_cap();
  std::vector<float> all((size_t)slice * t->nranks);
  const void* src = t->peer_mode ? (const void*)reinterpret_cast<PeerWindow*>(t->peer_local)->raw : (const void*)t->raw.p;
  PFT_CUDA_TRY(cudaMemcpy(all.data(), src, all.size() * sizeof(float), cudaMemcpyDeviceToHost));
  for (size_t i = 0; i < n; ++i) out[i] = all[(i % t->nranks) * slice + i / t->nranks];
  return PFT_OK;
}

int pft_tracker_get_ancestors(pft_tracker* t, int32_t* out, size_t capacity, size_t* n_out) {
  if (!t) { set_last_error("null tracker"); return PFT_ERR_INVALID; }
  TrackerState h;
  int rc = read_state(t, &h);
  if (rc) return rc;
  const size_t n = t->has_particles ? (size_t)h.particle_num : 0;
  if (n_out) *n_out = n;
  if (n > capacity) { set_last_error("capacity %zu < %zu", capacity, n); return PFT_ERR_CAPACITY; }
  if (n == 0) return PFT_OK;
  PFT_CUDA_TRY(cudaMemcpy(out, t->ancestors.p, n * sizeof(int), cudaMemcpyDeviceToHost));
  return PFT_OK;
}

int pft_tracker_get_nn(pft_tracker* t, int particle, int32_t* idx, float* d2, size_t capacity) {
  if (!t || !idx || !d2) { set_last_error("null argument"); return PFT_ERR_INVALID; }
  if (particle < 0 || particle >= t->debug_nn || !t->dbg_idx.p) { set_last_error("particle %d was not recorded (PFT_DEBUG_NN = %d)", particle, t->debug_nn); return PFT_ERR_STATE; }
  if ((size_t)t->M > capacity) { set_last_error("capacity %zu < %d", capacity, t->M); return PFT_ERR_CAPACITY; }
  PFT_CUDA_TRY(cudaSetDevice(t->ctx->device));
  PFT_CUDA_TRY(cudaStreamSynchronize(t->run_stream()));
  PFT_CUDA_TRY(cudaMemcpy(idx, t->dbg_idx.as<int>() + (size_t)particle * t->M, (size_t)t->M * sizeof(int), cudaMemcpyDeviceToHost));
  PFT_CUDA_TRY(cudaMemcpy(d2, t->dbg_d2.as<float>() + (size_t)particle * t->M, (size_t)t->M * sizeof(float), cudaMemcpyDeviceToHost));
  return PFT_OK;
}

int pft_tracker_enable_timing(pft_tracker* t, int on) {
  if (!t) { set_last_error("null tracker"); return PFT_ERR_INVALID; }
  t->timing = on != 0;
  return PFT_OK;
}

int pft_tracker_get_timing(pft_tracker* t, float* weight_ms, float* compute_ms) {
  if (!t) { set_last_error("null tracker"); return PFT_ERR_INVALID; }
  if (!t->timing || !t->ev_c0) { set_last_error("timing is not enabled or no compute() has run"); return PFT_ERR_STATE; }
  PFT_CUDA_TRY(cudaSetDevice(t->ctx->device));
  PFT_CUDA_TRY(cudaStreamSynchronize(t->run_stream()));
  float w = 0.f;
  for (int k = 0; k < t->n_ev_used; ++k) {
    float ms = 0.f;
    PFT_CUDA_TRY(cudaEventElapsedTime(&ms, t->ev_w[2 * k], t->ev_w[2 * k + 1]));
    w += ms;
  }
  float c = 0.f;
  if (cudaEventElapsedTime(&c, t->ev_c0, t->ev_c1) != cudaSuccess) { cudaGetLastError(); c = 0.f; }
  if (weight_ms) *weight_ms = w;
  if (compute_ms) *compute_ms = c;
  return PFT_OK;
}

int pft_tracker_get_kernel_times(pft_tracker* t, const char** names, float* ms, int capacity, int* n_out) {
  if (!t) { set_last_error("null tracker"); return PFT_ERR_INVALID; }
  if (!t->timing || !t->ev_c0) { set_last_error("timing is not enabled or no compute() has run"); return PFT_ERR_STATE; }
  PFT_CUDA_TRY(cudaSetDevice(t->ctx->device));
  PFT_CUDA_TRY(cudaStreamSynchronize(t->run_stream()));
  if (n_out) *n_out = t->n_ev_k;
  if (t->n_ev_k > capacity) { set_last_error("capacity %d < %d", capacity, t->n_ev_k); return PFT_ERR_CAPACITY; }
  for (int k = 0; k < t->n_ev_k; ++k) {
    float v = 0.f;
    if (cudaEventElapsedTime(&v, k ? t->ev_k[k - 1] : t->ev_c0, t->ev_k[k]) != cudaSuccess) { cudaGetLastError(); v = 0.f; }
    if (names) names[k] = t->ev_k_name[k];
    if (ms) ms[k] = v;
  }
  return PFT_OK;
}

int pft_tracker_weight_phase(pft_tracker* t, int phase) {
  if (!t) { set_last_error("null tracker"); return PFT_ERR_INVALID; }
// ... 398 lines not shown
```

pcl_tracking_b200/csrc/pft_tracker_kernels.cuh:

```cuda
#pragma once
#include <cooperative_groups.h>

#include "pft_common.cuh"

namespace pft {

#ifdef PFT_TRACE
__device__ unsigned long long g_trace[64];
__device__ __forceinline__ unsigned long long trace_now() { unsigned long long t; asm volatile("mov.u64 %0, %globaltimer;" : "=l"(t)); return t; }
#define PFT_TRACE_MIN(i) do { if ((threadIdx.x & 31) == 0) atomicMin(&g_trace[i], trace_now()); } while (0)
#define PFT_TRACE_MAX(i) do { if ((threadIdx.x & 31) == 0) atomicMax(&g_trace[i], trace_now()); } while (0)
#else
#define PFT_TRACE_MIN(i)
#define PFT_TRACE_MAX(i)
#endif
struct TrackerState {
  int particle_num;
  int has_particles;
  float aabb[6];
  DevParticle rep;
  DevParticle motion;
  double fit_ratio;
  double weight_sum;
  unsigned long long draw_call;
  unsigned long long nn_sum_um, nn_count;
  unsigned int peer_epoch;
  unsigned int peer_error;
  int resample_n_old;
  unsigned int work_counter;
  unsigned long long evals;
  unsigned int aabb_blocks_done;
};

constexpr int kMaxPeers = 16;
struct PeerWindow {
  float box[2][kMaxPeers][8];
  unsigned int flag_box;
  unsigned int flag_raw;
  unsigned int pad[30];
  float raw[1];
};
struct PeerSet {
  PeerWindow* win[kMaxPeers];
  int nranks, rank;
};

__device__ __forceinline__ bool peer_wait(volatile unsigned int* flag, unsigned int target, unsigned int* error) {
  const long long t0 = clock64();
  while ((int)(*flag - target) < 0) {
    if (clock64() - t0 > 8000000000ll) { *error = 1u; return false; }
    __nanosleep(64);
  }
  __threadfence_system();
  return true;
}

__device__ __forceinline__ void peer_box_exchange(TrackerState* st, const PeerSet& ps) {
  const int lane = threadIdx.x & 31;
  PeerWindow* me = ps.win[ps.rank];
  unsigned int e = 0;
  if (lane == 0) { e = st->peer_epoch + 1u; st->peer_epoch = e; }
  e = __shfl_sync(kFull, e, 0);
  const int cur = e & 1u;
  for (int r0 = 0; r0 < ps.nranks; r0 += 4) {
    const int r = r0 + (lane >> 3), d = lane & 7;
    if (r < ps.nranks && d < 6) ps.win[r]->box[cur][ps.rank][d] = __ldcg(&st->aabb[d]);
  }
  __syncwarp();
  if (lane == 0) __threadfence_system();
  __syncwarp();
  if (lane < ps.nranks) atomicAdd_system(&ps.win[lane]->flag_box, 1u);
  bool ok = true;
  if (lane == 0) ok = peer_wait(&me->flag_box, e * (unsigned int)ps.nranks, &st->peer_error);
  ok = __shfl_sync(kFull, ok, 0);
  if (!ok) return;
  if (lane < 6) {
    float v = __ldcg(&me->box[cur][0][lane]);
    for (int r = 1; r < ps.nranks; ++r) {
      const float o = __ldcg(&me->box[cur][r][lane]);
      v = lane < 3 ? fminf(v, o) : fmaxf(v, o);
    }
    st->aabb[lane] = v;
  }
}

struct CloudPeerSet {
  float4* pts[kMaxPeers];
  CloudHeader* hdr[kMaxPeers];
  unsigned int* sync[kMaxPeers];
  int nranks, rank;
};
__global__ void __launch_bounds__(256) cloud_push_kernel(const float4* __restrict__ src, const CloudHeader* __restrict__ src_hdr, CloudPeerSet ps,
                                                         unsigned int epoch, int capacity, unsigned int* error ) {
  int n = src_hdr->n;
  if (n > capacity) { if (blockIdx.x == 0 && threadIdx.x == 0) *error = 1u; n = 0; }
  for (int i = blockIdx.x * blockDim.x + threadIdx.x; i < n; i += gridDim.x * blockDim.x) {
    const float4 p = src[i];
    for (int r = 0; r < ps.nranks; ++r) if (r != ps.rank) ps.pts[r][i] = p;
  }
  if (blockIdx.x == 0 && threadIdx.x < ps.nranks && (int)threadIdx.x != ps.rank) { CloudHeader h = *src_hdr; h.n = n; *ps.hdr[threadIdx.x] = h; }
  __syncthreads();
  if (threadIdx.x == 0) {
    __threadfence_system();
    unsigned int* mine = ps.sync[ps.rank];
    if (atomicAdd(&mine[1], 1u) + 1u == gridDim.x) {
      mine[1] = 0u;
      __threadfence_system();
      for (int r = 0; r < ps.nranks; ++r) if (r != ps.rank) atomicExch_system(&ps.sync[r][0], epoch);
    }
  }
}
__global__ void cloud_wait_kernel(unsigned int* sync, unsigned int epoch, unsigned int* error ) {
  peer_wait(&sync[0], epoch, error);
}
// ... 195 lines not shown
        if (lane == 0) {
#pragma unroll
          for (int d = 0; d < 3; ++d) { s_red[wid][d] = mn[d]; s_red[wid][3 + d] = mx[d]; }
        }
        __syncthreads();
#pragma unroll
        for (int w = 0; w < WARPS; ++w) {
#pragma unroll
          for (int d = 0; d < 3; ++d) { mn[d] = fminf(mn[d], s_red[w][d]); mx[d] = fmaxf(mx[d], s_red[w][3 + d]); }
        }
      }
      if (wid == 0) {
        if (lane < 3) slot_aabb[(size_t)s * 6 + lane] = mn[lane];
        else if (lane < 6) slot_aabb[(size_t)s * 6 + lane] = mx[lane - 3];
      }
    }
#pragma unroll
    for (int d = 0; d < 3; ++d) { un[d] = fminf(un[d], mn[d]); ux[d] = fmaxf(ux[d], mx[d]); }
  }
  if (wid == 0 && un[0] <= ux[0]) {
    if (lane < 3) atomic_min_float(&st->aabb[lane], un[lane]);
    else if (lane < 6) atomic_max_float(&st->aabb[lane], ux[lane - 3]);
  }
  if (peer_exchange && wid == 0) {
    unsigned int done = 0;
    __syncwarp();
    if (lane == 0) { __threadfence(); done = atomicAdd(&st->aabb_blocks_done, 1u) + 1u; }
    done = __shfl_sync(kFull, done, 0);
    if (done == gridDim.x) {
      if (lane == 0) { st->aabb_blocks_done = 0u; __threadfence(); }
      __syncwarp();
      peer_box_exchange(st, ps);
    }
  }
}

__device__ inline void compute_index_header(const float* crop, const float* aabb , float inv_leaf,
                                            int base_level, int max_cells, IndexHeader& h) {
#pragma unroll
  for (int d = 0; d < 6; ++d) { h.aabb[d] = crop[d]; h.built[d] = aabb[d]; h.core[d] = crop[d]; }
  h.reuse = 0; h.n_in_crop = 0; h.dilate = 0.f;
  h.inv_leaf = inv_leaf;
  h.n_cropped = 0;
  h.valid = (crop[0] <= crop[3] && crop[1] <= crop[4] && crop[2] <= crop[5]) ? 1 : 0;
  h.level = base_level; h.level_scale = 1.0f; h.n_cells = 0;
  h.dim[0] = h.dim[1] = h.dim[2] = 0; h.origin[0] = h.origin[1] = h.origin[2] = 0;
  h.cell = 1.0f / inv_leaf;
  h.f_cells = 0; h.use_lists = 0;
  h.f_origin[0] = h.f_origin[1] = h.f_origin[2] = 0; h.f_dim[0] = h.f_dim[1] = h.f_dim[2] = 0;
  if (!h.valid) return;
  float lo[3], hi[3];
#pragma unroll
  for (int d = 0; d < 3; ++d) { lo[d] = aabb[d] * inv_leaf; hi[d] = aabb[3 + d] * inv_leaf; }
  {
    long long fc = 1;
#pragma unroll
    for (int d = 0; d < 3; ++d) {
      h.f_origin[d] = (int)floorf(lo[d]);
      h.f_dim[d] = (int)floorf(hi[d]) - h.f_origin[d] + 1;
      fc *= (long long)h.f_dim[d];
      if (fc > (1ll << 30)) fc = 1ll << 30;
    }
    h.f_cells = (int)fc;
  }
  for (int level = base_level; level < 24; ++level) {
    const float ls = 1.0f / (float)(1 << level);
    int dim[3], org[3];
#pragma unroll
    for (int d = 0; d < 3; ++d) {
      org[d] = (int)floorf(lo[d] * ls);
      dim[d] = (int)floorf(hi[d] * ls) - org[d] + 1;
    }
    const long long cells = (long long)dim[0] * dim[1] * dim[2];
    if (cells <= (long long)max_cells || level == 23) {
      h.level = level; h.level_scale = ls; h.n_cells = (int)min(cells, (long long)max_cells);
#pragma unroll
      for (int d = 0; d < 3; ++d) { h.dim[d] = dim[d]; h.origin[d] = org[d]; }
      h.cell = (float)(1 << level) / inv_leaf;
      break;
    }
  }
}

__global__ void index_begin_kernel(TrackerState* st, IndexHeader* hdr, int* cell_count, float inv_leaf, int max_cells,
                                   int list_max_cells, int M, int nranks, int rank, unsigned int* needed_words,
                                   int* list_counters ,
                                   unsigned int* built_bits , int reuse_allowed, float dilate,
                                   int list_ratio ,
                                   const IndexHeader* __restrict__ hdr_prev ) {
  __shared__ IndexHeader h;
  PFT_TRACE_MIN(0);
  if (threadIdx.x == 0) {
    const IndexHeader old = *hdr_prev;
    bool reuse = reuse_allowed && old.valid && old.use_lists && old.n_cropped < 65535;
    if (reuse) {
      reuse = st->aabb[0] <= st->aabb[3] && st->aabb[1] <= st->aabb[4] && st->aabb[2] <= st->aabb[5];
#pragma unroll
      for (int d = 0; d < 3; ++d) reuse = reuse && st->aabb[d] >= old.built[d] && st->aabb[3 + d] <= old.built[3 + d];
      if (old.core[0] <= old.core[3] && old.core[1] <= old.core[4] && old.core[2] <= old.core[5]) {
#pragma unroll
        for (int d = 0; d < 3; ++d) reuse = reuse && st->aabb[d] <= old.core[d] && st->aabb[3 + d] >= old.core[3 + d];
      }
    }
    if (reuse) {
      h = old;
#pragma unroll
      for (int d = 0; d < 6; ++d) h.aabb[d] = st->aabb[d];
      h.reuse = 1; h.n_in_crop = 0; h.epoch = old.epoch + 1u;
#pragma unroll
      for (int d = 0; d < 3; ++d) { h.core[d] = fminf(old.core[d], st->aabb[d] + old.dilate); h.core[3 + d] = fmaxf(old.core[3 + d], st->aabb[3 + d] - old.dilate); }
    } else {
      int base_level = 1;
      if (st->nn_count > 0) {
        const float mean_d = (float)((double)st->nn_sum_um / (double)st->nn_count) * 1.0e-6f;
        const float want = mean_d * 1.15f * inv_leaf;
        base_level = want <= 1.5f ? 1 : (want <= 3.0f ? 1 : (want <= 6.0f ? 2 : (want <= 12.0f ? 3 : 4)));
      }
      const int n = st->particle_num;
      const long long n_local = n > rank ? (n - rank + nranks - 1) / nranks : 0;
      float box[6];
#pragma unroll
      for (int d = 0; d < 6; ++d) box[d] = st->aabb[d];
      compute_index_header(st->aabb, box, inv_leaf, base_level, max_cells, h);
      bool lists = h.valid && h.f_cells > 0 && h.f_cells <= list_max_cells && (M == 0 || n_local * (long long)M >= (long long)list_ratio * h.f_cells);
      if (lists && dilate > 0.f) {
        IndexHeader hd;
#pragma unroll
        for (int d = 0; d < 3; ++d) { box[d] = st->aabb[d] - dilate; box[3 + d] = st->aabb[3 + d] + dilate; }
        compute_index_header(st->aabb, box, inv_leaf, base_level, max_cells, hd);
        if (hd.f_cells > 0 && hd.f_cells <= list_max_cells) {
          h = hd;
          h.dilate = dilate;
#pragma unroll
          for (int d = 0; d < 3; ++d) { h.core[d] = st->aabb[d] + dilate; h.core[3 + d] = st->aabb[3 + d] - dilate; }
        }
      }
      h.use_lists = lists ? 1 : 0;
      h.epoch = old.epoch + 1u;
    }
    if (blockIdx.x == 0) *hdr = h;
  }
  __syncthreads();
  if (!h.reuse) {
    const int nc = h.n_cells + 1;
    for (int i = blockIdx.x * blockDim.x + threadIdx.x; i < nc; i += gridDim.x * blockDim.x) cell_count[i] = 0;
  }
  if (h.use_lists) {
    for (int i = blockIdx.x * blockDim.x + threadIdx.x; i < h.f_cells; i += gridDim.x * blockDim.x) needed_words[i] = 0u;
    if (!h.reuse) {
      const int words = (h.f_cells + 31) >> 5;
      for (int i = blockIdx.x * blockDim.x + threadIdx.x; i < words; i += gridDim.x * blockDim.x) built_bits[i] = 0u;
    }
  }
  if (blockIdx.x == 0 && threadIdx.x == 0) {
    if (!h.reuse) { list_counters[0] = 0; list_counters[3] = 0; }
    list_counters[1] = 0; list_counters[2] = 0; list_counters[4] = 0;
    st->work_counter = 0u;
  }
}

__device__ __forceinline__ bool in_built(const float4& p, const IndexHeader& h) {
  return isfinite(p.x) && isfinite(p.y) && isfinite(p.z) && p.x >= h.built[0] && p.x <= h.built[3] && p.y >= h.built[1] &&
         p.y <= h.built[4] && p.z >= h.built[2] && p.z <= h.built[5];
}
constexpr unsigned int kInCropBit = 0x80000000u;
__device__ __forceinline__ bool in_crop(const float4& p, const IndexHeader& h) {
  return isfinite(p.x) && isfinite(p.y) && isfinite(p.z) && p.x >= h.aabb[0] && p.x <= h.aabb[3] && p.y >= h.aabb[1] &&
         p.y <= h.aabb[4] && p.z >= h.aabb[2] && p.z <= h.aabb[5];
}
__device__ __forceinline__ int cell_of(const float4& p, const IndexHeader& h) {
  const int cx = (int)floorf((p.x * h.inv_leaf) * h.level_scale) - h.origin[0];
  const int cy = (int)floorf((p.y * h.inv_leaf) * h.level_scale) - h.origin[1];
  const int cz = (int)floorf((p.z * h.inv_leaf) * h.level_scale) - h.origin[2];
  return (cz * h.dim[1] + cy) * h.dim[0] + cx;
}

__global__ void index_count_kernel(const float4* __restrict__ scene, const CloudHeader* __restrict__ scene_hdr, IndexHeader* hdr, int* cell_count,
                                   float4* __restrict__ pts2) {
  __shared__ IndexHeader h;
  if (threadIdx.x == 0) h = *hdr;
  __syncthreads();
  if (!h.valid) return;
  if (h.reuse) {
    int local = 0;
    for (int i = blockIdx.x * blockDim.x + threadIdx.x; i < h.n_cropped; i += gridDim.x * blockDim.x) {
      float4 p = pts2[i];
      const bool in = in_crop(p, h);
      const unsigned int w = (__float_as_uint(p.w) & ~kInCropBit) | (in ? kInCropBit : 0u);
      if (w != __float_as_uint(p.w)) pts2[i].w = __uint_as_float(w);
      local += in ? 1 : 0;
    }
    local = warp_sum(local);
    if ((threadIdx.x & 31) == 0 && local) atomicAdd(&hdr->n_in_crop, local);
    return;
  }
  const int ns = scene_hdr->n;
  int local = 0, local_in = 0;
  for (int i = blockIdx.x * blockDim.x + threadIdx.x; i < ns; i += gridDim.x * blockDim.x) {
    const float4 p = scene[i];
    if (!in_built(p, h)) continue;
    atomicAdd(&cell_count[cell_of(p, h)], 1);
    ++local;
    local_in += in_crop(p, h) ? 1 : 0;
  }
  local = warp_sum(local);
  local_in = warp_sum(local_in);
  if ((threadIdx.x & 31) == 0 && local) { atomicAdd(&hdr->n_cropped, local); atomicAdd(&hdr->n_in_crop, local_in); }
}

__global__ void __launch_bounds__(1024) index_scan_kernel(const IndexHeader* __restrict__ hdr, int* cell_count, int* __restrict__ cell_start,
                                                          TrackerState* st, float4* __restrict__ pts, float4* __restrict__ pts2, IndexHeader* hdr_prev) {
  __shared__ int smem[34];
  const int nc = hdr->n_cells;
  if (threadIdx.x == 0) {
    st->nn_sum_um = 0ull; st->nn_count = 0ull;
    *hdr_prev = *hdr;
  }
  if (hdr->reuse) return;
  const int total = block_exclusive_scan<int>(
      nc, [&](int i) { return cell_count[i]; }, [&](int i, int ex) { cell_start[i] = ex; cell_count[i] = 0; }, smem);
  if (threadIdx.x == 0) {
    cell_start[nc] = total;
    pts[total] = make_float4(3.0e38f, 3.0e38f, 3.0e38f, __int_as_float(0x7fffffff));
    pts2[total] = make_float4(3.0e38f, 3.0e38f, 3.0e38f, 0.f);
  }
}

__global__ void index_scatter_kernel(const float4* __restrict__ scene, const CloudHeader* __restrict__ scene_hdr, const IndexHeader* __restrict__ hdr,
                                     const int* __restrict__ cell_start, int* cell_count, float4* __restrict__ pts, unsigned int* __restrict__ hsv,
                                     float4* __restrict__ pts2 ) {
  __shared__ IndexHeader h;
  if (threadIdx.x == 0) h = *hdr;
  __syncthreads();
  if (!h.valid || h.reuse) return;
  const int ns = scene_hdr->n;
  for (int i = blockIdx.x * blockDim.x + threadIdx.x; i < ns; i += gridDim.x * blockDim.x) {
    const float4 p = scene[i];
    if (!in_built(p, h)) continue;
    const int c = cell_of(p, h);
    const int pos = cell_start[c] + atomicAdd(&cell_count[c], 1);
    pts[pos] = make_float4(p.x, p.y, p.z, __int_as_float(i));
    const unsigned int packed = rgba_to_hsv_packed(__float_as_uint(p.w));
    hsv[pos] = packed;
    pts2[pos] = make_float4(p.x, p.y, p.z, __uint_as_float(packed | (in_crop(p, h) ? kInCropBit : 0u)));
  }
}

#ifdef PFT_STATS
__device__ unsigned long long g_stats[48];
#define PFT_STAT(i, v) atomicAdd(&g_stats[i], (unsigned long long)(v))
#else
#define PFT_STAT(i, v)
#endif
constexpr int kRT = 11;
constexpr int kRows = (2 * kRT + 1) * (2 * kRT + 1);
struct RowEntry { signed char dy, dz; unsigned short lb2; };

struct NNResult {
  float dist2;
  int orig_idx;
  int slot;
  __device__ __forceinline__ float d2() const { return dist2; }
  __device__ __forceinline__ int orig() const { return orig_idx; }
};
__device__ __forceinline__ NNResult nn_none(float lim2) { return NNResult{lim2, (int)0x80000000, -1}; }

__device__ __forceinline__ void nn_eval(const IndexHeader& h, const float4* __restrict__ pts, int slot, float qx, float qy, float qz, NNResult& best) {
  const float4 p = pts[slot];
  if (!(p.x >= h.aabb[0] && p.x <= h.aabb[3] && p.y >= h.aabb[1] && p.y <= h.aabb[4] && p.z >= h.aabb[2] && p.z <= h.aabb[5])) return;
  const float dx = qx - p.x, dy = qy - p.y, dz = qz - p.z;
  const float d2 = (dx * dx + dy * dy) + dz * dz;
  const int orig = __float_as_int(p.w);
  if (d2 < best.dist2 || (d2 == best.dist2 && orig < best.orig_idx)) { best.dist2 = d2; best.orig_idx = orig; best.slot = slot; }
}

__device__ __forceinline__ float axis_gap(int d, float t) {
  const float g = d > 0 ? (float)d - t : (d < 0 ? t - (float)(d + 1) : 0.f);
  return fmaxf(g - 2.5e-4f, 0.f);
}

template <typename CS>
__device__ __noinline__ NNResult nn_search_shells(const CS* __restrict__ cs, const float4* __restrict__ pts, const IndexHeader& h, float qx, float qy,
                                                  float qz, int cx, int cy, int cz, float tx, float ty, float tz, float lim2, NNResult best) {
  const float tmin = fminf(fminf(fminf(tx, 1.f - tx), fminf(ty, 1.f - ty)), fminf(tz, 1.f - tz));
  const float cell2 = h.cell * h.cell;
  int r_prev = kRT, r = kRT + 1;
  while (true) {
    const float done = ((float)r_prev + tmin - 2.5e-4f) * h.cell;
    const bool covered = (cx - r_prev <= 0) && (cx + r_prev >= h.dim[0] - 1) && (cy - r_prev <= 0) && (cy + r_prev >= h.dim[1] - 1) &&
                         (cz - r_prev <= 0) && (cz + r_prev >= h.dim[2] - 1);
    if (covered || done * done * 0.9999f > fminf(best.d2(), lim2)) return best;
    const int z0 = max(cz - r, 0), z1 = min(cz + r, h.dim[2] - 1);
    const int y0 = max(cy - r, 0), y1 = min(cy + r, h.dim[1] - 1);
    for (int z = z0; z <= z1; ++z) {
      const int dz = z - cz;
      const float az = axis_gap(dz, tz);
      for (int y = y0; y <= y1; ++y) {
        const int dy = y - cy;
        const float ay = axis_gap(dy, ty);
        if ((az * az + ay * ay) * cell2 * 0.9999f > best.d2()) continue;
        const int base = (z * h.dim[1] + y) * h.dim[0];
        const bool inner = max(abs(dy), abs(dz)) <= r_prev;
        for (int seg = 0; seg < 2; ++seg) {
          int xa, xb;
          if (!inner) { if (seg) break; xa = cx - r; xb = cx + r; }
          else if (seg == 0) { xa = cx - r; xb = cx - r_prev - 1; }
          else { xa = cx + r_prev + 1; xb = cx + r; }
          xa = max(xa, 0); xb = min(xb, h.dim[0] - 1);
          if (xa > xb) continue;
          const int s1 = (int)cs[base + xb + 1];
          for (int s = (int)cs[base + xa]; s < s1; ++s) nn_eval(h, pts, s, qx, qy, qz, best);
        }
      }
    }
    r_prev = r;
    int need = 2 * r;
    if (best.slot >= 0) need = max(r + 1, (int)ceilf(sqrtf(best.d2()) / h.cell - tmin + 0.004f));
    const int rcap = max(r + 1, (int)ceilf(sqrtf(lim2) / h.cell - tmin + 0.004f));
    r = min(need, rcap);
  }
}

template <typename CS>
__device__ __forceinline__ NNResult nn_search(const CS* __restrict__ cs, const float4* __restrict__ pts, const IndexHeader& h,
// ... 1411 lines not shown
  const float* mats;
  double* partial;
  int chunks, chunk_len, n_max, nranks, rank_id;
  CoherenceParams co;
  int dbg_k; int* dbg_idx; float* dbg_d2;
};

__global__ void __launch_bounds__(256) weight_approx_kernel(const WeightApproxArgs a) {
  __shared__ OctHeaderD H;
  if (threadIdx.x == 0) H = *a.oct;
  __syncthreads();
  const int n = a.st->particle_num;
  const int n_local = n > a.rank_id ? (n - a.rank_id + a.nranks - 1) / a.nranks : 0;
  const int items = n_local * a.chunks;
  const int lane = threadIdx.x & 31;
  const int warp = (blockIdx.x * blockDim.x + threadIdx.x) >> 5, nwarps = (gridDim.x * blockDim.x) >> 5;
  for (int item = warp; item < items; item += nwarps) {
    const int il = item / a.chunks, c = item - il * a.chunks;
    const int i = a.rank_id + il * a.nranks;
    float m[12];
    {
      const float4* mp = reinterpret_cast<const float4*>(a.mats) + (size_t)i * 3;
      const float4 r0 = mp[0], r1 = mp[1], r2 = mp[2];
      m[0] = r0.x; m[1] = r0.y; m[2] = r0.z; m[3] = r0.w; m[4] = r1.x; m[5] = r1.y; m[6] = r1.z; m[7] = r1.w;
      m[8] = r2.x; m[9] = r2.y; m[10] = r2.z; m[11] = r2.w;
    }
    const int j0 = c * a.chunk_len, j1 = min(a.M, j0 + a.chunk_len);
    double val = 0.0;
    for (int j = j0 + lane; j < j1; j += 32) {
      const float4 mp = a.model[j];
      float qx, qy, qz, d2 = FLT_MAX;
      xform(m, mp.x, mp.y, mp.z, qx, qy, qz);
      int idx = H.overflow ? -1 : octree_approx_nearest(H, a.nodes, a.next, a.scene, qx, qy, qz, d2);
      if (idx < 0) d2 = FLT_MAX;
      if (i < a.dbg_k) {
        const size_t o = (size_t)i * a.M + a.model_perm[j];
        a.dbg_idx[o] = idx;
        a.dbg_d2[o] = d2;
      }
      if (idx >= 0 && (double)d2 < a.co.max_d2) {
        double den = 1.0;
        if (a.co.use_dist) { const double d = (double)sqrtf(d2); den = 1.0 + d * d * a.co.dist_w; }
        if (a.co.use_hsv) {
          const unsigned int sb = __float_as_uint(mp.w), tb = rgba_to_hsv_packed(__float_as_uint(a.scene[idx].w));
          const float sh = (float)(sb & 0xff) / 180.0f, ss = (float)((sb >> 8) & 0xff) / 255.0f, sv = (float)((sb >> 16) & 0xff) / 255.0f;
          const float th = (float)(tb & 0xff) / 180.0f, ts = (float)((tb >> 8) & 0xff) / 255.0f, tv = (float)((tb >> 16) & 0xff) / 255.0f;
          const float hd = fabsf(sh - th);
          float hd2;
          if (sh < th) hd2 = fabsf(1.0f + sh - th); else hd2 = fabsf(1.0f + th - sh);
          float h_diff;
          if (hd < hd2) h_diff = a.co.h_w * hd * hd; else h_diff = a.co.h_w * hd2 * hd2;
          const float s_diff = a.co.s_w * (ss - ts) * (ss - ts);
          const float v_diff = a.co.v_w * (sv - tv) * (sv - tv);
          den *= 1.0 + a.co.hsv_w * (double)(h_diff + s_diff + v_diff);
        }
        val += 1.0 / den;
      }
    }
    val = warp_sum(val);
    if (lane == 0) a.partial[(size_t)c * a.n_max + i] = val;
  }
}

__device__ __forceinline__ int raw_slot(int i, int nranks, int slice_cap) { return (i % nranks) * slice_cap + i / nranks; }

__global__ void weights_to_raw_kernel(const TrackerState* st, const DevParticle* __restrict__ parts, float* __restrict__ raw, int nranks, int slice_cap) {
  const int n = st->particle_num;
  for (int i = blockIdx.x * blockDim.x + threadIdx.x; i < n; i += gridDim.x * blockDim.x) raw[raw_slot(i, nranks, slice_cap)] = parts[i].weight;
}

__device__ __forceinline__ float raw_weight(const double* __restrict__ partial, int chunks, int n_max, int i) {
  double v = 0.0;
  for (int c = 0; c < chunks; ++c) v += partial[(size_t)c * n_max + i];
  return -(float)v;
}

__global__ void raw_weights_kernel(const TrackerState* st, const double* __restrict__ partial, int chunks, int n_max,
                                   float* __restrict__ raw, int slice_cap, int nranks, int rank) {
  const int n = st->particle_num;
  for (int l = blockIdx.x * blockDim.x + threadIdx.x; rank + l * nranks < n; l += gridDim.x * blockDim.x)
    raw[rank * slice_cap + l] = raw_weight(partial, chunks, n_max, rank + l * nranks);
}

namespace cg = cooperative_groups;
constexpr int kClusterCtas = 8;

template <int CTAS, typename Particle>
__device__ __forceinline__ void update_state(TrackerState* st, int n, Particle particle, double* red6 ,
                                             double* s_part ) {
  cg::cluster_group cluster = cg::this_cluster();
  const unsigned int crank = cluster.block_rank();
  double acc[6] = {0, 0, 0, 0, 0, 0};
  for (int i = crank * blockDim.x + threadIdx.x; i < n; i += CTAS * blockDim.x) {
    const DevParticle p = particle(i);
    const double w = (double)p.weight;
    acc[0] += (double)(float)((double)p.x * w); acc[1] += (double)(float)((double)p.y * w); acc[2] += (double)(float)((double)p.z * w);
    acc[3] += (double)(float)((double)p.roll * w); acc[4] += (double)(float)((double)p.pitch * w); acc[5] += (double)(float)((double)p.yaw * w);
  }
  block_sum6(acc, red6);
  if (threadIdx.x == 0) {
#pragma unroll
    for (int d = 0; d < 6; ++d) s_part[d] = acc[d];
  }
  cluster.sync();
  if (crank == 0 && threadIdx.x == 0) {
    double tot[6] = {0, 0, 0, 0, 0, 0};
    for (int r = 0; r < CTAS; ++r) {
      const double* p = cluster.map_shared_rank(s_part, r);
      for (int d = 0; d < 6; ++d) tot[d] += p[d];
    }
    const DevParticle o = st->rep;
    DevParticle r{(float)tot[0], (float)tot[1], (float)tot[2], 1.f, (float)tot[3], (float)tot[4], (float)tot[5], 1.0f / (float)n};
    st->rep = r;
    st->motion = DevParticle{r.x - o.x, r.y - o.y, r.z - o.z, 1.f, r.roll - o.roll, r.pitch - o.pitch, r.yaw - o.yaw, 0.f};
  }
}

template <int CTAS>
__global__ void __cluster_dims__(CTAS, 1, 1) __launch_bounds__(1024)
normalize_kernel(TrackerState* st, DevParticle* parts, float* raw , double alpha, int nranks,
                 int slice_cap, const CloudHeader* __restrict__ scene_hdr, int M,
                 const double* __restrict__ partial ,
                 int chunks, int n_max, int fuse_update ,
                 PeerSet ps ) {
  cg::cluster_group cluster = cg::this_cluster();
  const unsigned int crank = cluster.block_rank();
  PFT_TRACE_MIN(11);
  __shared__ double red[32];
  __shared__ double s_part[3];
  __shared__ double s_upd[6];
  __shared__ double red6[192];
  if (partial && ps.nranks > 1) {
    const int np = st->particle_num;
    for (int l = crank * blockDim.x + threadIdx.x; ps.rank + l * nranks < np; l += CTAS * blockDim.x) {
      const float w = raw_weight(partial, chunks, n_max, ps.rank + l * nranks);
      for (int r = 0; r < nranks; ++r) ps.win[r]->raw[ps.rank * slice_cap + l] = w;
    }
    cluster.sync();
    if (crank == 0 && threadIdx.x == 0) {
      __threadfence_system();
      for (int r = 0; r < nranks; ++r) atomicAdd_system(&ps.win[r]->flag_raw, 1u);
      peer_wait(&ps.win[ps.rank]->flag_raw, st->peer_epoch * (unsigned int)nranks, &st->peer_error);
    }
    cluster.sync();
    raw = ps.win[ps.rank]->raw;
    partial = nullptr;
  }
  if (scene_hdr->n <= 0) return;
  const int n = st->particle_num;
  const int lane = threadIdx.x & 31, wid = threadIdx.x >> 5, nw = blockDim.x >> 5;
  const int first = crank * blockDim.x + threadIdx.x, stride = CTAS * blockDim.x;
  double wmin = DBL_MAX, wmax = -DBL_MAX;
  for (int i = first; i < n; i += stride) {
    double w;
    if (partial) {
      const float wf = raw_weight(partial, chunks, n_max, i);
      raw[i] = wf;
      w = (double)wf;
    } else {
      w = (double)__ldcg(&raw[raw_slot(i, nranks, slice_cap)]);
    }
    if (wmin > w) wmin = w;
    if (w != 0.0 && wmax < w) wmax = w;
  }
  for (int o = 16; o > 0; o >>= 1) { wmin = fmin(wmin, __shfl_xor_sync(kFull, wmin, o)); wmax = fmax(wmax, __shfl_xor_sync(kFull, wmax, o)); }
  if (lane == 0) { red[wid] = wmin; red6[wid] = wmax; }
  __syncthreads();
  if (threadIdx.x < 2) {
// ... 462 lines not shown
```

pcl_tracking_b200/pcl.py:

```python
import ctypes as C

import numpy as np

from . import _capi as capi
from ._capi import PARTICLE, POINT, POINT_PCL32, PftError, check, ptr


class Context:

    _default = {}

    def __init__(self, device=0):
        self._h = C.c_void_p()
        check(capi.load().pft_context_create(int(device), C.byref(self._h)))
        self.device = int(device)

    @classmethod
    def default(cls, device=0):
        if device not in cls._default:
            cls._default[device] = cls(device)
        return cls._default[device]

    def synchronize(self):
        check(capi.load().pft_context_synchronize(self._h))
# ... 535 lines not shown
        check(capi.load().pft_tracker_get_motion(self._h, ptr(out)))
        return out[0]

    def injectDraws(self, usel, normals6, umotion):
        if usel is None:
            check(capi.load().pft_tracker_inject_draws(self._h, None, None, None, 0, 0))
            return
        usel = np.ascontiguousarray(usel, dtype=np.float32)
        slots, stride = usel.shape
        normals6 = np.ascontiguousarray(normals6, dtype=np.float32).reshape(slots, stride, 6)
        umotion = np.ascontiguousarray(umotion, dtype=np.float32).reshape(slots, stride)
        check(capi.load().pft_tracker_inject_draws(self._h, ptr(usel), ptr(normals6), ptr(umotion), slots, stride))

    def seed(self, s):
        check(capi.load().pft_tracker_seed(self._h, int(s)))

    def setSampler(self, s):
        self._si(capi.SAMPLER, s)

    def setQuaternionSampling(self, on):
        self._si(capi.QUAT_SAMPLE, 1 if on else 0)

    def setCandidateLists(self, mode):
        self._si(capi.CANDIDATE_LISTS, mode)

    def setDebugNN(self, k):
        self._si(capi.DEBUG_NN, k)

    def setChanged(self, c):
        check(capi.load().pft_tracker_set_changed(self._h, 1 if c else 0))

    def initParticles(self):
        check(capi.load().pft_tracker_init_particles(self._h))

    def resample(self, slot=0):
        check(capi.load().pft_tracker_resample(self._h, int(slot)))

    def weight(self):
        check(capi.load().pft_tracker_weight(self._h))

    def weightPhase(self, phase):
        check(capi.load().pft_tracker_weight_phase(self._h, int(phase)))

    def update(self):
        check(capi.load().pft_tracker_update(self._h))

    def aabb(self):
        a = np.zeros(6, dtype=np.float32)
        check(capi.load().pft_tracker_get_aabb(self._h, ptr(a)))
        return a

    def cropBox(self):
        a = np.zeros(6, dtype=np.float32)
        check(capi.load().pft_tracker_get_crop_box(self._h, ptr(a)))
        return a

    def setCropBox(self, a):
        a = np.ascontiguousarray(a, dtype=np.float32)
        check(capi.load().pft_tracker_set_crop_box(self._h, ptr(a)))

    def rawSlice(self, rank):
        n = C.c_size_t()
        capi.load().pft_tracker_get_raw_slice(self._h, int(rank), None, 0, C.byref(n))
        out = np.zeros(n.value, dtype=np.float32)
        check(capi.load().pft_tracker_get_raw_slice(self._h, int(rank), ptr(out), n.value, C.byref(n)))
        return out

    def setRawSlice(self, rank, values):
        a = np.ascontiguousarray(values, dtype=np.float32)
        check(capi.load().pft_tracker_set_raw_slice(self._h, int(rank), ptr(a), a.shape[0]))

    def setShard(self, nranks, rank):
        check(capi.load().pft_tracker_set_shard(self._h, int(nranks), int(rank)))

    def croppedCount(self):
        n = C.c_size_t()
        check(capi.load().pft_tracker_get_cropped_count(self._h, C.byref(n)))
        return n.value

    def indexInfo(self):
        a = np.zeros(8, dtype=np.int32)
        check(capi.load().pft_tracker_get_index_info(self._h, ptr(a)))
        return dict(zip(("dim_x", "dim_y", "dim_z", "level", "n_cropped", "n_cells", "use_lists", "list_cells"), a.tolist()))

    def rawWeights(self):
        n = C.c_size_t()
        rc = capi.load().pft_tracker_get_raw_weights(self._h, None, 0, C.byref(n))
        if rc not in (capi.OK, capi.ERR_CAPACITY):
            check(rc)
        out = np.zeros(n.value, dtype=np.float32)
        if n.value:
            check(capi.load().pft_tracker_get_raw_weights(self._h, ptr(out), n.value, C.byref(n)))
        return out

    def ancestors(self):
        n = C.c_size_t()
        rc = capi.load().pft_tracker_get_ancestors(self._h, None, 0, C.byref(n))
        if rc not in (capi.OK, capi.ERR_CAPACITY):
            check(rc)
        out = np.zeros(n.value, dtype=np.int32)
        if n.value:
            check(capi.load().pft_tracker_get_ancestors(self._h, ptr(out), n.value, C.byref(n)))
        return out

    def nn(self, particle, m):
        idx = np.zeros(m, dtype=np.int32)
        d2 = np.zeros(m, dtype=np.float32)
        check(capi.load().pft_tracker_get_nn(self._h, int(particle), ptr(idx), ptr(d2), m))
        return idx, d2

    def enableTiming(self, on=True):
        check(capi.load().pft_tracker_enable_timing(self._h, 1 if on else 0))

    def timing(self):
        w, c = C.c_float(), C.c_float()
        check(capi.load().pft_tracker_get_timing(self._h, C.byref(w), C.byref(c)))
        return w.value, c.value

    def kernelTimes(self):
        cap = 256
        names = (C.c_char_p * cap)()
        ms = (C.c_float * cap)()
        n = C.c_int()
        check(capi.load().pft_tracker_get_kernel_times(self._h, names, ms, cap, C.byref(n)))
        return [(names[i].decode(), float(ms[i])) for i in range(n.value)]

    def evalCount(self):
        n = C.c_uint64()
        check(capi.load().pft_tracker_get_eval_count(self._h, C.byref(n)))
        return n.value

    def graphReplays(self):
        n = C.c_uint64()
        check(capi.load().pft_tracker_graph_replays(self._h, C.byref(n)))
        return n.value

    def commInit(self, nranks, rank, unique_id):
        buf = (C.c_char * 128).from_buffer_copy(bytes(unique_id))
        check(capi.load().pft_tracker_comm_init(self._h, int(nranks), int(rank), buf))

    def commDestroy(self):
        check(capi.load().pft_tracker_comm_destroy(self._h))

    def setDevices(self, devices):
        arr = (C.c_int * len(devices))(*[int(d) for d in devices])
        check(capi.load().pft_tracker_set_devices(self._h, len(devices), arr))

    def follower(self, rank):
        v = object.__new__(type(self))
        v.ctx, v._input, v._h = self.ctx, None, C.c_void_p()
        check(capi.load().pft_tracker_get_follower(self._h, int(rank), C.byref(v._h)))
        v._borrowed = True
        return v

    def peerExport(self):
        buf = C.create_string_buffer(capi.PEER_HANDLE_BYTES)
        check(capi.load().pft_tracker_peer_export(self._h, buf))
        return bytes(buf.raw)

    def peerAttach(self, handles):
        blob = b"".join(bytes(h) for h in handles)
        buf = C.create_string_buffer(blob, len(blob))
        check(capi.load().pft_tracker_peer_attach(self._h, buf))

    def peerDetach(self):
        check(capi.load().pft_tracker_peer_detach(self._h))
# ... 84 lines not shown
```

Before: 7.493 billion.

## Fuse spatial index count/scan/scatter into cluster kernel and decoupled-lookback voxel rank

The scene spatial index build previously ran three kernels: atomic cell counting, a single-block scan, and an atomic scatter. Counting and per-point slot ordering now happen inside index_begin, and one 8-CTA cluster kernel scans cell counts through distributed shared memory and then scatters points using the precomputed order. Separately, the voxel-grid filter's tile count, scan and assign kernels are replaced by a single kernel using a decoupled-lookback prefix scan. Both changes cut kernel launches and global round-trips. The trade-off is that the scatter now runs on only 8 CTAs, which may limit bandwidth on a large scene, and a debug index-dump API is also added.

```diff
diff --git a/include/pft/pft.h b/include/pft/pft.h
--- a/include/pft/pft.h
+++ b/include/pft/pft.h
@@ -156,6 +156,8 @@
 PFT_API int pft_tracker_get_kernel_times(pft_tracker* t, const char** names, float* ms, int capacity, int* n);
 
 PFT_API int pft_tracker_get_index_info(pft_tracker* t, int* info8);
+PFT_API int pft_tracker_get_index(pft_tracker* t, int* ints8, float* geom14, int* cell_start, size_t cell_cap, float* points,
+                                  unsigned int* staged, size_t point_cap);
 PFT_API int pft_tracker_graph_replays(pft_tracker* t, uint64_t* n);
 
 PFT_API int pft_tracker_weight_phase(pft_tracker* t, int phase);
diff --git a/pcl_tracking_b200/_capi.py b/pcl_tracking_b200/_capi.py
--- a/pcl_tracking_b200/_capi.py
+++ b/pcl_tracking_b200/_capi.py
@@ -105,6 +105,7 @@
     "pft_tracker_enable_timing": (_i, [_vp, _i]),
     "pft_tracker_get_kernel_times": (_i, [_vp, _vp, _vp, _i, C.POINTER(C.c_int)]),
     "pft_tracker_get_index_info": (_i, [_vp, _vp]),
+    "pft_tracker_get_index": (_i, [_vp, _vp, _vp, _vp, _sz, _vp, _vp, _sz]),
     "pft_tracker_graph_replays": (_i, [_vp, C.POINTER(C.c_uint64)]),
     "pft_tracker_weight_phase": (_i, [_vp, _i]),
     "pft_tracker_get_crop_box": (_i, [_vp, _vp]),
diff --git a/pcl_tracking_b200/csrc/pft_filters.cu b/pcl_tracking_b200/csrc/pft_filters.cu
--- a/pcl_tracking_b200/csrc/pft_filters.cu
+++ b/pcl_tracking_b200/csrc/pft_filters.cu
@@ -74,7 +74,9 @@
 }
 
 __global__ void k1_insert_kernel(const float4* __restrict__ in, const CloudHeader* __restrict__ in_hdr, unsigned long long* keys,
-                                 int* first, int* __restrict__ slot_of, unsigned int mask, float inv, int field, float lo, float hi) {
+                                 int* first, int* __restrict__ slot_of, unsigned int mask, float inv, int field, float lo, float hi,
+                                 unsigned long long* __restrict__ tile_state, int n_tiles) {
+  for (int t = blockIdx.x * blockDim.x + threadIdx.x; t <= n_tiles; t += gridDim.x * blockDim.x) tile_state[t] = 0ull;
   const int n = in_hdr->n;
   for (int i = blockIdx.x * blockDim.x + threadIdx.x; i < n; i += gridDim.x * blockDim.x) {
     const float4 p = in[i];
@@ -94,42 +96,26 @@
   }
 }
 constexpr int kTile = 4096;
+constexpr unsigned long long kTileAggregate = 1ull << 32;
+constexpr unsigned long long kTileInclusive = 2ull << 32;
 
 __device__ __forceinline__ int k1_is_first(int i, int n, const int* __restrict__ slot_of, const int* __restrict__ first) {
   if (i >= n) return 0;
   const int s = slot_of[i];
   return (s >= 0 && first[s] == i) ? 1 : 0;
 }
-__global__ void __launch_bounds__(1024) k1_tile_count_kernel(const CloudHeader* __restrict__ in_hdr, const int* __restrict__ slot_of,
-                                                             const int* __restrict__ first, int* __restrict__ tile_count) {
-  __shared__ int red[32];
-  const int n = in_hdr->n;
-  const int base = blockIdx.x * kTile + threadIdx.x * 4;
-  int c = 0;
-#pragma unroll
-  for (int k = 0; k < 4; ++k) c += k1_is_first(base + k, n, slot_of, first);
-  c = warp_sum(c);
-  if ((threadIdx.x & 31) == 0) red[threadIdx.x >> 5] = c;
+__global__ void __launch_bounds__(1024) k1_rank_kernel(const CloudHeader* __restrict__ in_hdr, const int* __restrict__ slot_of,
+                                                       const int* __restrict__ first, int n_tiles,
+                                                       unsigned long long* tile_state ,
+                                                       int* __restrict__ vid, CloudHeader* out_hdr) {
+  __shared__ int wsum[32];
+  __shared__ int s_tile, s_before;
+  if (threadIdx.x == 0) s_tile = (int)atomicAdd(&tile_state[n_tiles], 1ull);
   __syncthreads();
-  if (threadIdx.x < 32) {
-    int v = red[threadIdx.x];
-    v = warp_sum(v);
-    if (threadIdx.x == 0) tile_count[blockIdx.x] = v;
-  }
-}
-__global__ void __launch_bounds__(1024) k1_tile_scan_kernel(int n_tiles, int* tile_count, CloudHeader* out_hdr) {
-  __shared__ int smem[34];
-  const int total = block_exclusive_scan<int>(
-      n_tiles, [&](int i) { return tile_count[i]; }, [&](int i, int ex) { tile_count[i] = ex; }, smem);
-  if (threadIdx.x == 0) out_hdr->n = total;
-}
-__global__ void __launch_bounds__(1024) k1_tile_assign_kernel(const CloudHeader* __restrict__ in_hdr, const int* __restrict__ slot_of,
-                                                              const int* __restrict__ first, const int* __restrict__ tile_offset,
-                                                              int* __restrict__ vid, double* acc_xyz, unsigned int* acc_rgbc) {
-  __shared__ int wsum[32];
+  const int tile = s_tile;
   const int n = in_hdr->n;
   const int lane = threadIdx.x & 31, wid = threadIdx.x >> 5;
-  const int base = blockIdx.x * kTile + threadIdx.x * 4;
+  const int base = tile * kTile + threadIdx.x * 4;
   int f[4], sum = 0;
 #pragma unroll
   for (int k = 0; k < 4; ++k) { f[k] = k1_is_first(base + k, n, slot_of, first); sum += f[k]; }
@@ -144,9 +130,27 @@
 #pragma unroll
     for (int o = 1; o < 32; o <<= 1) { const int t = __shfl_up_sync(kFull, winc, o); if (lane >= o) winc += t; }
     wsum[lane] = winc - w;
+    const int count = __shfl_sync(kFull, winc, 31);
+    volatile unsigned long long* state = tile_state;
+    if (lane == 0) state[tile] = (tile == 0 ? kTileInclusive : kTileAggregate) | (unsigned int)count;
+    int before = 0;
+    for (int j = tile - 1; j >= 0;) {
+      const unsigned long long v = j - lane >= 0 ? (unsigned long long)state[j - lane] : kTileInclusive;
+      if (__any_sync(kFull, (v >> 32) == 0ull)) continue;
+      const unsigned int incl = __ballot_sync(kFull, (v >> 32) == 2ull);
+      const int last = incl ? __ffs(incl) - 1 : 31;
+      before += warp_sum(lane <= last ? (int)(unsigned int)v : 0);
+      if (incl) break;
+      j -= 32;
+    }
+    if (lane == 0) {
+      if (tile > 0) state[tile] = kTileInclusive | (unsigned int)(before + count);
+      if (tile == n_tiles - 1) out_hdr->n = before + count;
+      s_before = before;
+    }
   }
   __syncthreads();
-  int ex = tile_offset[blockIdx.x] + wsum[wid] + (inc - sum);
+  int ex = s_before + wsum[wid] + (inc - sum);
 #pragma unroll
   for (int k = 0; k < 4; ++k) {
     if (f[k]) {
@@ -291,14 +295,10 @@
   const float inv = 1.0f / leaf;
   const int grid = grid_for(cap, 256, ctx->sm_count);
   k1_insert_kernel<<<grid, 256, 0, s>>>(in->d_pts(), in->d_hdr(), ctx->k1_keys.as<unsigned long long>(), ctx->k1_first.as<int>(),
-                                        ctx->k1_slot_of.as<int>(), (unsigned int)(H - 1), inv, field, lo, hi);
-  PFT_LAUNCH_CHECK();
-  k1_tile_count_kernel<<<n_tiles, 1024, 0, s>>>(in->d_hdr(), ctx->k1_slot_of.as<int>(), ctx->k1_first.as<int>(), ctx->k1_blk.as<int>());
-  PFT_LAUNCH_CHECK();
-  k1_tile_scan_kernel<<<1, 1024, 0, s>>>(n_tiles, ctx->k1_blk.as<int>(), out->d_hdr());
-  PFT_LAUNCH_CHECK();
-  k1_tile_assign_kernel<<<n_tiles, 1024, 0, s>>>(in->d_hdr(), ctx->k1_slot_of.as<int>(), ctx->k1_first.as<int>(), ctx->k1_blk.as<int>(),
-                                                 ctx->k1_vid.as<int>(), ctx->k1_acc_xyz.as<double>(), ctx->k1_acc_rgbc.as<unsigned int>());
+                                        ctx->k1_slot_of.as<int>(), (unsigned int)(H - 1), inv, field, lo, hi, ctx->k1_blk.as<unsigned long long>(), n_tiles);
+  PFT_LAUNCH_CHECK();
+  k1_rank_kernel<<<n_tiles, 1024, 0, s>>>(in->d_hdr(), ctx->k1_slot_of.as<int>(), ctx->k1_first.as<int>(), n_tiles, ctx->k1_blk.as<unsigned long long>(),
+                                          ctx->k1_vid.as<int>(), out->d_hdr());
   PFT_LAUNCH_CHECK();
   k1_accum_kernel<<<grid, 256, 0, s>>>(in->d_pts(), in->d_hdr(), ctx->k1_slot_of.as<int>(), ctx->k1_vid.as<int>(),
                                        ctx->k1_acc_xyz.as<double>(), ctx->k1_acc_rgbc.as<unsigned int>());
@@ -323,7 +323,7 @@
   if ((rc = ctx->k1_acc_xyz.reserve(cap * 3 * sizeof(double)))) return rc;
   if ((rc = ctx->k1_acc_rgbc.reserve(cap * 4 * sizeof(unsigned int)))) return rc;
   const int n_tiles = (int)((cap + kTile - 1) / kTile);
-  if ((rc = ctx->k1_blk.reserve((size_t)n_tiles * sizeof(int)))) return rc;
+  if ((rc = ctx->k1_blk.reserve((size_t)(n_tiles + 1) * sizeof(unsigned long long)))) return rc;
   out->host_n = -1;
   (void)kFirstInit;
   static const bool use_graph = [] { const char* e = getenv("PFT_NO_GRAPH"); return !(e && e[0] == '1'); }();
@@ -355,7 +355,7 @@
     ctx->k1_key[slot] = key;
   }
   PFT_CUDA_TRY(cudaGraphLaunch(ctx->k1_exec[slot], ctx->stream));
-  g_launch_count += 6;
+  g_launch_count += 4;
   return PFT_OK;
 }
 
diff --git a/pcl_tracking_b200/csrc/pft_tracker.cu b/pcl_tracking_b200/csrc/pft_tracker.cu
--- a/pcl_tracking_b200/csrc/pft_tracker.cu
+++ b/pcl_tracking_b200/csrc/pft_tracker.cu
@@ -129,7 +129,7 @@
   unsigned long long graph_replays = 0;
   int graph_nodes[2] = {0, 0};
   DevBuf st, parts[2], mats, slot_aabb, model, model_perm, model_tmp, sort_keys, sort_idx, bbox, raw, partial, cdf, cdf_total, ancestors, bin_keys, tbl_rep,
-      tbl_min, slot_of, klb, d_usel, d_normals, d_umot, idx_hdr, idx_hdr_prev, fbuilt_bits, cell_start, ipts, ipts2, ihsv, icount, dbg_idx, dbg_d2, d_trans, row_table, flists, fpool, fcell_items, fl1_slots, fneeded, fneeded_list, ffar_list, xlists, xcount, result_box, alias_a, alias_q, alias_hl, oct_hdr, oct_nodes, oct_next, cd_hdr, cd_nodes, cd_out;
+      tbl_min, slot_of, klb, d_usel, d_normals, d_umot, idx_hdr, idx_hdr_prev, fbuilt_bits, cell_start, iorder, ipts, ipts2, ihsv, icount, dbg_idx, dbg_d2, d_trans, row_table, flists, fpool, fcell_items, fl1_slots, fneeded, fneeded_list, ffar_list, xlists, xcount, result_box, alias_a, alias_q, alias_hl, oct_hdr, oct_nodes, oct_next, cd_hdr, cd_nodes, cd_out;
   int oct_node_cap = 0;
   bool use_cd = false;
   int cd_interval = 10, cd_filter = 10, change_counter = 0, cd_tests = 0, cd_last_found = -1, cd_node_cap = 0, cd_resets = 0;
@@ -168,7 +168,7 @@
 void release_all(pft_tracker* t) {
   DevBuf* bufs[] = {&t->st, &t->parts[0], &t->parts[1], &t->mats, &t->slot_aabb, &t->model, &t->model_perm, &t->model_tmp, &t->sort_keys, &t->sort_idx,
                     &t->bbox, &t->raw, &t->partial, &t->cdf, &t->cdf_total, &t->ancestors, &t->bin_keys, &t->tbl_rep, &t->tbl_min, &t->slot_of, &t->klb,
-                    &t->d_usel, &t->d_normals, &t->d_umot, &t->idx_hdr, &t->idx_hdr_prev, &t->fbuilt_bits, &t->cell_start, &t->ipts, &t->ipts2, &t->ihsv, &t->icount, &t->dbg_idx,
+                    &t->d_usel, &t->d_normals, &t->d_umot, &t->idx_hdr, &t->idx_hdr_prev, &t->fbuilt_bits, &t->cell_start, &t->iorder, &t->ipts, &t->ipts2, &t->ihsv, &t->icount, &t->dbg_idx,
                     &t->dbg_d2, &t->d_trans, &t->row_table, &t->flists, &t->fpool, &t->fcell_items, &t->fl1_slots, &t->fneeded, &t->fneeded_list, &t->ffar_list, &t->xlists, &t->xcount, &t->result_box, &t->alias_a, &t->alias_q, &t->alias_hl, &t->oct_hdr, &t->oct_nodes, &t->oct_next, &t->cd_hdr, &t->cd_nodes, &t->cd_out};
   for (auto* b : bufs) b->release();
 }
@@ -288,6 +288,7 @@
     if ((rc = t->d_trans.reserve(12 * sizeof(float)))) return rc;
     if ((rc = t->cell_start.reserve(((size_t)t->max_cells + 16) * sizeof(int)))) return rc;
     if ((rc = t->icount.reserve(((size_t)t->max_cells + 16) * sizeof(int)))) return rc;
+    PFT_CUDA_TRY(cudaMemsetAsync(t->icount.p, 0, ((size_t)t->max_cells + 16) * sizeof(int), s));
     if ((rc = upload_row_table(t))) return rc;
     if (t->list_max_cells > 0) {
       if ((rc = t->flists.reserve(((size_t)t->list_max_cells + 1) * 8 * 8 * sizeof(unsigned int)))) return rc;
@@ -410,6 +411,7 @@
   if ((rc = t->ipts.reserve((cap + 4) * sizeof(float4)))) return rc;
   if ((rc = t->ipts2.reserve((cap + 4) * sizeof(float4)))) return rc;
   if ((rc = t->ihsv.reserve((cap + 4) * sizeof(unsigned int)))) return rc;
+  if ((rc = t->iorder.reserve((cap + 4) * sizeof(int2)))) return rc;
   t->scene_cap = cap;
   return PFT_OK;
 }
@@ -590,13 +592,14 @@
   return timed_lookup(t, "weight_approx_kernel", [&] { weight_approx_kernel<<<sm * 8, 256, 0, s>>>(w); });
 }
 
-int launch_index_begin(pft_tracker* t, bool reuse_allowed = false) {
+int launch_index_begin(pft_tracker* t, bool reuse_allowed, bool count_scene) {
   const int sm = t->ctx->sm_count;
   const float inv_leaf = 1.0f / (float)t->search_res;
   index_begin_kernel<<<sm, 256, 0, t->run_stream()>>>(t->st.as<TrackerState>(), t->idx_hdr.as<IndexHeader>(), t->icount.as<int>(), inv_leaf, t->max_cells,
                                                       t->list_mode ? t->list_max_cells : 0, t->list_mode == 2 ? 0 : t->M, t->nranks, t->rank,
                                                       t->fneeded.as<unsigned int>(), t->xcount.as<int>(), t->fbuilt_bits.as<unsigned int>(),
-                                                      reuse_allowed ? 1 : 0, t->iteration_num > 1 ? kIndexDilate : 0.f, kListRatio, t->idx_hdr_prev.as<IndexHeader>());
+                                                      reuse_allowed ? 1 : 0, t->iteration_num > 1 ? kIndexDilate : 0.f, kListRatio, t->idx_hdr_prev.as<IndexHeader>(),
+                                                      t->input->d_pts(), t->input->d_hdr(), t->iorder.as<int2>(), count_scene ? 1 : 0);
   PFT_LAUNCH_CHECK();
   stage_mark(t, "index_begin_kernel");
   return PFT_OK;
@@ -609,15 +612,18 @@
   const int sm = t->ctx->sm_count;
   TrackerState* st = t->st.as<TrackerState>();
   const pft_cloud* in = t->input;
-  const int ncap_scene = (int)std::max<size_t>(in->capacity, 1);
   IndexHeader* hdr = t->idx_hdr.as<IndexHeader>();
   const float inv_leaf = 1.0f / (float)t->search_res;
-  const int gscene = blocks_for(ncap_scene, 256, sm * 4);
   const bool lists = t->list_max_cells > 0 && t->list_mode && t->nn_mode == PFT_NN_EXACT;
-  if ((rc = launch_index_begin(t, reuse_allowed && lists))) return rc;
+  if ((rc = launch_index_begin(t, reuse_allowed && lists, true))) return rc;
+  if (lists) PFT_CUDA_TRY(cudaEventRecord(t->ev_fork, s));
+  index_build_kernel<<<kClusterCtas, kIndexBuildThreads, 0, s>>>(in->d_pts(), hdr, t->icount.as<int>(), t->cell_start.as<int>(), t->iorder.as<int2>(), st,
+                                                                 t->ipts.as<float4>(), t->ihsv.as<unsigned int>(), t->ipts2.as<float4>(),
+                                                                 t->idx_hdr_prev.as<IndexHeader>());
+  PFT_LAUNCH_CHECK();
+  stage_mark(t, "index_build_kernel");
   if (lists) {
     cudaStream_t sa = t->aux_stream;
-    PFT_CUDA_TRY(cudaEventRecord(t->ev_fork, s));
     PFT_CUDA_TRY(cudaStreamWaitEvent(sa, t->ev_fork, 0));
     const long long n_queries = (long long)std::max(1, (t->particle_num > 0 ? t->particle_num : t->n_cap) / t->nranks) * t->M;
     const size_t mark_smem = (size_t)(t->list_max_cells / 8 + 64);
@@ -628,16 +634,6 @@
     PFT_LAUNCH_CHECK();
     PFT_CUDA_TRY(cudaEventRecord(t->ev_join, sa));
   }
-  index_count_kernel<<<gscene, 256, 0, s>>>(in->d_pts(), in->d_hdr(), hdr, t->icount.as<int>(), t->ipts2.as<float4>());
-  PFT_LAUNCH_CHECK();
-  stage_mark(t, "index_count_kernel");
-  index_scan_kernel<<<1, 1024, 0, s>>>(hdr, t->icount.as<int>(), t->cell_start.as<int>(), st, t->ipts.as<float4>(), t->ipts2.as<float4>(), t->idx_hdr_prev.as<IndexHeader>());
-  PFT_LAUNCH_CHECK();
-  stage_mark(t, "index_scan_kernel");
-  index_scatter_kernel<<<gscene, 256, 0, s>>>(in->d_pts(), in->d_hdr(), hdr, t->cell_start.as<int>(), t->icount.as<int>(), t->ipts.as<float4>(),
-                                              t->ihsv.as<unsigned int>(), t->ipts2.as<float4>());
-  PFT_LAUNCH_CHECK();
-  stage_mark(t, "index_scatter_kernel");
   if (lists) {
     PFT_CUDA_TRY(cudaStreamWaitEvent(s, t->ev_join, 0));
     stage_mark(t, "cand_mark+collect (beside the index)");
@@ -705,7 +701,7 @@
 }
 
 int change_detection_test(pft_tracker* t, bool* change) {
-  int rc = launch_index_begin(t);
+  int rc = launch_index_begin(t, false, false);
   if (rc) return rc;
   cudaStream_t s = t->run_stream();
   for (int attempt = 0; attempt < 2; ++attempt) {
@@ -1156,9 +1152,7 @@
       (const void*)cloud_wait_kernel,
       (const void*)draws_kernel,
       (const void*)index_begin_kernel,
-      (const void*)index_count_kernel,
-      (const void*)index_scan_kernel,
-      (const void*)index_scatter_kernel,
+      (const void*)index_build_kernel,
       (const void*)init_particles_kernel,
       (const void*)kld_insert_kernel,
       (const void*)kld_stop_kernel,
@@ -1537,6 +1531,34 @@
   return PFT_OK;
 }
 
+int pft_tracker_get_index(pft_tracker* t, int* ints8, float* geom14, int* cell_start, size_t cell_cap, float* points, unsigned int* staged,
+                          size_t point_cap) {
+  if (!t) { set_last_error("null tracker"); return PFT_ERR_INVALID; }
+  if (!t->idx_hdr.p) { set_last_error("no weight() has run"); return PFT_ERR_STATE; }
+  PFT_CUDA_TRY(cudaSetDevice(t->ctx->device));
+  cudaStream_t s = t->run_stream();
+  PFT_CUDA_TRY(cudaMemcpyAsync(t->ctx->pinned, t->idx_hdr.p, sizeof(IndexHeader), cudaMemcpyDeviceToHost, s));
+  PFT_CUDA_TRY(cudaStreamSynchronize(s));
+  const IndexHeader h = *reinterpret_cast<IndexHeader*>(t->ctx->pinned);
+  if (ints8) {
+    const int v[8] = {h.n_cropped, h.n_in_crop, h.n_cells, h.reuse, h.origin[0], h.origin[1], h.origin[2], h.valid};
+    memcpy(ints8, v, sizeof(v));
+  }
+  if (geom14) {
+    memcpy(geom14, h.aabb, 6 * sizeof(float));
+    memcpy(geom14 + 6, h.built, 6 * sizeof(float));
+    geom14[12] = h.inv_leaf; geom14[13] = h.level_scale;
+  }
+  const size_t nc = (size_t)h.n_cells + 1, np_ = (size_t)h.n_cropped;
+  if ((cell_start && cell_cap < nc) || ((points || staged) && point_cap < np_)) { set_last_error("capacity too small"); return PFT_ERR_CAPACITY; }
+  if (cell_start) PFT_CUDA_TRY(cudaMemcpyAsync(cell_start, t->cell_start.p, nc * sizeof(int), cudaMemcpyDeviceToHost, s));
+  if (points && np_) PFT_CUDA_TRY(cudaMemcpyAsync(points, t->ipts.p, np_ * sizeof(float4), cudaMemcpyDeviceToHost, s));
+  if (staged && np_)
+    PFT_CUDA_TRY(cudaMemcpy2DAsync(staged, sizeof(unsigned int), (const char*)t->ipts2.p + 12, sizeof(float4), sizeof(unsigned int), np_, cudaMemcpyDeviceToHost, s));
+  PFT_CUDA_TRY(cudaStreamSynchronize(s));
+  return PFT_OK;
+}
+
 int pft_tracker_get_raw_weights(pft_tracker* t, float* out, size_t capacity, size_t* n_out) {
   if (!t) { set_last_error("null tracker"); return PFT_ERR_INVALID; }
   TrackerState h;
diff --git a/pcl_tracking_b200/csrc/pft_tracker_kernels.cuh b/pcl_tracking_b200/csrc/pft_tracker_kernels.cuh
--- a/pcl_tracking_b200/csrc/pft_tracker_kernels.cuh
+++ b/pcl_tracking_b200/csrc/pft_tracker_kernels.cuh
@@ -14,6 +14,8 @@
 #define PFT_TRACE_MIN(i)
 #define PFT_TRACE_MAX(i)
 #endif
+namespace cg = cooperative_groups;
+constexpr int kClusterCtas = 8;
 struct TrackerState {
   int particle_num;
   int has_particles;
@@ -30,6 +32,7 @@
   unsigned int work_counter;
   unsigned long long evals;
   unsigned int aabb_blocks_done;
+  int index_points, index_in_crop;
 };
 
 constexpr int kMaxPeers = 16;
@@ -391,12 +394,32 @@
   }
 }
 
+__device__ __forceinline__ bool in_built(const float4& p, const IndexHeader& h) {
+  return isfinite(p.x) && isfinite(p.y) && isfinite(p.z) && p.x >= h.built[0] && p.x <= h.built[3] && p.y >= h.built[1] &&
+         p.y <= h.built[4] && p.z >= h.built[2] && p.z <= h.built[5];
+}
+constexpr unsigned int kInCropBit = 0x80000000u;
+__device__ __forceinline__ bool in_crop(const float4& p, const IndexHeader& h) {
+  return isfinite(p.x) && isfinite(p.y) && isfinite(p.z) && p.x >= h.aabb[0] && p.x <= h.aabb[3] && p.y >= h.aabb[1] &&
+         p.y <= h.aabb[4] && p.z >= h.aabb[2] && p.z <= h.aabb[5];
+}
+__device__ __forceinline__ int cell_of(const float4& p, const IndexHeader& h) {
+  const int cx = (int)floorf((p.x * h.inv_leaf) * h.level_scale) - h.origin[0];
+  const int cy = (int)floorf((p.y * h.inv_leaf) * h.level_scale) - h.origin[1];
+  const int cz = (int)floorf((p.z * h.inv_leaf) * h.level_scale) - h.origin[2];
+  return (cz * h.dim[1] + cy) * h.dim[0] + cx;
+}
+
+constexpr int kIndexBatch = 4;
 __global__ void index_begin_kernel(TrackerState* st, IndexHeader* hdr, int* cell_count, float inv_leaf, int max_cells,
                                    int list_max_cells, int M, int nranks, int rank, unsigned int* needed_words,
                                    int* list_counters ,
                                    unsigned int* built_bits , int reuse_allowed, float dilate,
                                    int list_ratio ,
-                                   const IndexHeader* __restrict__ hdr_prev ) {
+                                   const IndexHeader* __restrict__ hdr_prev ,
+                                   const float4* __restrict__ scene, const CloudHeader* __restrict__ scene_hdr,
+                                   int2* __restrict__ order ,
+                                   int count_scene ) {
   __shared__ IndexHeader h;
   PFT_TRACE_MIN(0);
   if (threadIdx.x == 0) {
@@ -450,9 +473,33 @@
     if (blockIdx.x == 0) *hdr = h;
   }
   __syncthreads();
-  if (!h.reuse) {
-    const int nc = h.n_cells + 1;
-    for (int i = blockIdx.x * blockDim.x + threadIdx.x; i < nc; i += gridDim.x * blockDim.x) cell_count[i] = 0;
+  if (count_scene && h.valid && !h.reuse) {
+    const int ns = scene_hdr->n;
+    const int lane = threadIdx.x & 31, stride = gridDim.x * blockDim.x;
+    int local_in = 0;
+    for (int w0 = blockIdx.x * blockDim.x + threadIdx.x - lane; w0 < ns; w0 += kIndexBatch * stride) {
+      float4 p[kIndexBatch];
+#pragma unroll
+      for (int k = 0; k < kIndexBatch; ++k) {
+        const int i = w0 + k * stride + lane;
+        p[k] = i < ns ? scene[i] : make_float4(NAN, NAN, NAN, 0.f);
+      }
+#pragma unroll
+      for (int k = 0; k < kIndexBatch; ++k) {
+        const bool in = in_built(p[k], h);
+        const unsigned int ballot = __ballot_sync(kFull, in);
+        if (!ballot) continue;
+        int base = 0;
+        if (lane == 0) base = atomicAdd(&st->index_points, __popc(ballot));
+        base = __shfl_sync(kFull, base, 0);
+        if (in) {
+          order[base + __popc(ballot & ((1u << lane) - 1u))] = make_int2(w0 + k * stride + lane, atomicAdd(&cell_count[cell_of(p[k], h)], 1));
+          local_in += in_crop(p[k], h) ? 1 : 0;
+        }
+      }
+    }
+    local_in = warp_sum(local_in);
+    if (lane == 0 && local_in) atomicAdd(&st->index_in_crop, local_in);
   }
   if (h.use_lists) {
     for (int i = blockIdx.x * blockDim.x + threadIdx.x; i < h.f_cells; i += gridDim.x * blockDim.x) needed_words[i] = 0u;
@@ -468,31 +515,25 @@
   }
 }
 
-__device__ __forceinline__ bool in_built(const float4& p, const IndexHeader& h) {
-  return isfinite(p.x) && isfinite(p.y) && isfinite(p.z) && p.x >= h.built[0] && p.x <= h.built[3] && p.y >= h.built[1] &&
-         p.y <= h.built[4] && p.z >= h.built[2] && p.z <= h.built[5];
-}
-constexpr unsigned int kInCropBit = 0x80000000u;
-__device__ __forceinline__ bool in_crop(const float4& p, const IndexHeader& h) {
-  return isfinite(p.x) && isfinite(p.y) && isfinite(p.z) && p.x >= h.aabb[0] && p.x <= h.aabb[3] && p.y >= h.aabb[1] &&
-         p.y <= h.aabb[4] && p.z >= h.aabb[2] && p.z <= h.aabb[5];
-}
-__device__ __forceinline__ int cell_of(const float4& p, const IndexHeader& h) {
-  const int cx = (int)floorf((p.x * h.inv_leaf) * h.level_scale) - h.origin[0];
-  const int cy = (int)floorf((p.y * h.inv_leaf) * h.level_scale) - h.origin[1];
-  const int cz = (int)floorf((p.z * h.inv_leaf) * h.level_scale) - h.origin[2];
-  return (cz * h.dim[1] + cy) * h.dim[0] + cx;
-}
-
-__global__ void index_count_kernel(const float4* __restrict__ scene, const CloudHeader* __restrict__ scene_hdr, IndexHeader* hdr, int* cell_count,
-                                   float4* __restrict__ pts2) {
+constexpr int kIndexBuildThreads = 512;
+__global__ void __cluster_dims__(kClusterCtas, 1, 1) __launch_bounds__(kIndexBuildThreads)
+index_build_kernel(const float4* __restrict__ scene, IndexHeader* hdr, int* cell_count, int* cell_start,
+                   const int2* __restrict__ order , TrackerState* st,
+                   float4* __restrict__ pts, unsigned int* __restrict__ hsv,
+                   float4* __restrict__ pts2 ,
+                   IndexHeader* hdr_prev) {
+  cg::cluster_group cluster = cg::this_cluster();
+  const unsigned int crank = cluster.block_rank();
   __shared__ IndexHeader h;
+  __shared__ int smem[34];
+  __shared__ int s_total;
   if (threadIdx.x == 0) h = *hdr;
   __syncthreads();
-  if (!h.valid) return;
-  if (h.reuse) {
+  const int first = crank * blockDim.x + threadIdx.x, stride = kClusterCtas * blockDim.x;
+  const int n_cropped = h.reuse ? h.n_cropped : st->index_points, n_in_crop = st->index_in_crop;
+  if (h.valid && h.reuse) {
     int local = 0;
-    for (int i = blockIdx.x * blockDim.x + threadIdx.x; i < h.n_cropped; i += gridDim.x * blockDim.x) {
+    for (int i = first; i < n_cropped; i += stride) {
       float4 p = pts2[i];
       const bool in = in_crop(p, h);
       const unsigned int w = (__float_as_uint(p.w) & ~kInCropBit) | (in ? kInCropBit : 0u);
@@ -501,54 +542,46 @@
     }
     local = warp_sum(local);
     if ((threadIdx.x & 31) == 0 && local) atomicAdd(&hdr->n_in_crop, local);
-    return;
-  }
-  const int ns = scene_hdr->n;
-  int local = 0, local_in = 0;
-  for (int i = blockIdx.x * blockDim.x + threadIdx.x; i < ns; i += gridDim.x * blockDim.x) {
-    const float4 p = scene[i];
-    if (!in_built(p, h)) continue;
-    atomicAdd(&cell_count[cell_of(p, h)], 1);
-    ++local;
-    local_in += in_crop(p, h) ? 1 : 0;
-  }
-  local = warp_sum(local);
-  local_in = warp_sum(local_in);
-  if ((threadIdx.x & 31) == 0 && local) { atomicAdd(&hdr->n_cropped, local); atomicAdd(&hdr->n_in_crop, local_in); }
-}
-
-__global__ void __launch_bounds__(1024) index_scan_kernel(const IndexHeader* __restrict__ hdr, int* cell_count, int* __restrict__ cell_start,
-                                                          TrackerState* st, float4* __restrict__ pts, float4* __restrict__ pts2, IndexHeader* hdr_prev) {
-  __shared__ int smem[34];
-  const int nc = hdr->n_cells;
-  if (threadIdx.x == 0) {
+  }
+  cluster.sync();
+  if (crank == 0 && threadIdx.x == 0) {
     st->nn_sum_um = 0ull; st->nn_count = 0ull;
-    *hdr_prev = *hdr;
-  }
-  if (hdr->reuse) return;
-  const int total = block_exclusive_scan<int>(
-      nc, [&](int i) { return cell_count[i]; }, [&](int i, int ex) { cell_start[i] = ex; cell_count[i] = 0; }, smem);
-  if (threadIdx.x == 0) {
+    IndexHeader snap = h;
+    if (h.reuse) {
+      snap.n_in_crop = __ldcg(&hdr->n_in_crop);
+    } else {
+      snap.n_cropped = hdr->n_cropped = n_cropped;
+      snap.n_in_crop = hdr->n_in_crop = n_in_crop;
+      st->index_points = 0; st->index_in_crop = 0;
+    }
+    *hdr_prev = snap;
+  }
+  if (h.reuse) return;
+  const int nc = h.n_cells;
+  const int seg = (nc + kClusterCtas - 1) / kClusterCtas;
+  const int c0 = min((int)crank * seg, nc), c1 = min(c0 + seg, nc);
+  const int mine = block_exclusive_scan<int>(
+      c1 - c0, [&](int c) { return cell_count[c0 + c]; }, [&](int c, int ex) { cell_start[c0 + c] = ex; cell_count[c0 + c] = 0; }, smem);
+  if (threadIdx.x == 0) s_total = mine;
+  cluster.sync();
+  int before = 0, total = 0;
+  for (int r = 0; r < kClusterCtas; ++r) {
+    const int v = *cluster.map_shared_rank(&s_total, r);
+    if (r < (int)crank) before += v;
+    total += v;
+  }
+  if (before) for (int c = c0 + threadIdx.x; c < c1; c += blockDim.x) cell_start[c] += before;
+  if (crank == 0 && threadIdx.x == 0) {
     cell_start[nc] = total;
     pts[total] = make_float4(3.0e38f, 3.0e38f, 3.0e38f, __int_as_float(0x7fffffff));
     pts2[total] = make_float4(3.0e38f, 3.0e38f, 3.0e38f, 0.f);
   }
-}
-
-__global__ void index_scatter_kernel(const float4* __restrict__ scene, const CloudHeader* __restrict__ scene_hdr, const IndexHeader* __restrict__ hdr,
-                                     const int* __restrict__ cell_start, int* cell_count, float4* __restrict__ pts, unsigned int* __restrict__ hsv,
-                                     float4* __restrict__ pts2 ) {
-  __shared__ IndexHeader h;
-  if (threadIdx.x == 0) h = *hdr;
-  __syncthreads();
-  if (!h.valid || h.reuse) return;
-  const int ns = scene_hdr->n;
-  for (int i = blockIdx.x * blockDim.x + threadIdx.x; i < ns; i += gridDim.x * blockDim.x) {
-    const float4 p = scene[i];
-    if (!in_built(p, h)) continue;
-    const int c = cell_of(p, h);
-    const int pos = cell_start[c] + atomicAdd(&cell_count[c], 1);
-    pts[pos] = make_float4(p.x, p.y, p.z, __int_as_float(i));
+  cluster.sync();
+  for (int e = first; e < n_cropped; e += stride) {
+    const int2 o = order[e];
+    const float4 p = scene[o.x];
+    const int pos = __ldcg(&cell_start[cell_of(p, h)]) + o.y;
+    pts[pos] = make_float4(p.x, p.y, p.z, __int_as_float(o.x));
     const unsigned int packed = rgba_to_hsv_packed(__float_as_uint(p.w));
     hsv[pos] = packed;
     pts2[pos] = make_float4(p.x, p.y, p.z, __uint_as_float(packed | (in_crop(p, h) ? kInCropBit : 0u)));
@@ -2126,8 +2159,6 @@
     raw[rank * slice_cap + l] = raw_weight(partial, chunks, n_max, rank + l * nranks);
 }
 
-namespace cg = cooperative_groups;
-constexpr int kClusterCtas = 8;
 
 template <int CTAS, typename Particle>
 __device__ __forceinline__ void update_state(TrackerState* st, int n, Particle particle, double* red6 ,
diff --git a/pcl_tracking_b200/pcl.py b/pcl_tracking_b200/pcl.py
--- a/pcl_tracking_b200/pcl.py
+++ b/pcl_tracking_b200/pcl.py
@@ -641,6 +641,18 @@
         a = np.zeros(8, dtype=np.int32)
         check(capi.load().pft_tracker_get_index_info(self._h, ptr(a)))
         return dict(zip(("dim_x", "dim_y", "dim_z", "level", "n_cropped", "n_cells", "use_lists", "list_cells"), a.tolist()))
+
+    def indexDump(self):
+        ints, geom = np.zeros(8, dtype=np.int32), np.zeros(14, dtype=np.float32)
+        check(capi.load().pft_tracker_get_index(self._h, ptr(ints), ptr(geom), None, 0, None, None, 0))
+        n_cropped, n_in_crop, n_cells, reuse = (int(v) for v in ints[:4])
+        cell_start = np.zeros(n_cells + 1, dtype=np.int32)
+        points = np.zeros((n_cropped, 4), dtype=np.float32)
+        staged = np.zeros(n_cropped, dtype=np.uint32)
+        check(capi.load().pft_tracker_get_index(self._h, ptr(ints), ptr(geom), ptr(cell_start), cell_start.size, ptr(points), ptr(staged), n_cropped))
+        return {"n_cropped": n_cropped, "n_in_crop": n_in_crop, "n_cells": n_cells, "reuse": bool(reuse), "origin": ints[4:7].copy(),
+                "valid": bool(ints[7]), "crop": geom[:6].copy(), "built": geom[6:12].copy(), "inv_leaf": geom[12], "level_scale": geom[13],
+                "cell_start": cell_start, "xyz": points[:, :3].copy(), "input_index": points[:, 3].view(np.int32).copy(), "staged_word": staged}
 
     def rawWeights(self):
         n = C.c_size_t()
```

Result: faster. 7.596 billion (median of 6 runs) (+1.4%).
